# mcdiarmid/waveforms

Measured on AMD Instinct MI355X. Metric: SOQPSK-TG Msym/s mod+Viterbi-detect @8sps, higher is better.
Workload: dtype f64; 1 GPU; SOQPSK-TG 1e+07 symbols @8 sps, modulate + AWGN + PT matched filter + 4-state Viterbi detect (BASELINE configs[1]); waveform=soqpsk, sps=8, prbs=PN23, noise=Philox4x32-10 + Box-Muller (device), fuse=175, streams=1, detector_warmup_rows=16, detector_form=lanes (one chunk per lane), parallelism=independent trial blocks x1

## Files before the change

### include/wfhip.h

```cpp
#ifndef WFHIP_H
#define WFHIP_H

#include <stdint.h>

#ifdef __cplusplus
extern "C" {
#endif

typedef enum {
    WF_OK = 0,
    WF_ERR_VALUE = -1,
    WF_ERR_KEY = -2,
    WF_ERR_HIP = -3,
    WF_ERR_DEVICE = -4,
    WF_ERR_NOMEM = -5
} wf_status;

typedef struct wf_ctx wf_ctx;

const char *wf_version(void);
const char *wf_last_error_string(void);

int wf_ctx_create(int device, wf_ctx **out);
int wf_ctx_destroy(wf_ctx *ctx);
int wf_ctx_retire(wf_ctx *ctx);
int wf_ctx_check(wf_ctx *ctx, void *stream);
typedef enum {
    WF_OPT_CPM_FORM = 0,
    WF_OPT_CPM_CHUNK_CALLS = 1,
    WF_OPT_DET_REPAIR = 2,
    WF_OPT_DET_FINAL_VERIFY = 3,
    WF_OPT_ITERATION_SERVER = 4,
    WF_OPT_MCB_TAIL_PERMILLE = 5,
    WF_OPT_PIPE_RESERVE_CUS = 6,
    WF_OPT_CPM_SAMPLES_MIN_CALLS = 7,
    WF_OPT_SOFT_CHUNK_CALLS = 8,
    WF_OPT_CPM_SOFT_CHUNK_CALLS = 9,
    WF_OPT_COUNT = 10
} wf_option;
int wf_ctx_set_option(wf_ctx *ctx, int key, int64_t value);
int wf_ctx_get_option(wf_ctx *ctx, int key, int64_t *value);
int wf_ctx_forget_promises(wf_ctx *ctx);

int wf_lfsr_generate(wf_ctx *ctx, int degree, uint64_t mask, uint64_t state, uint64_t skip,
                     uint8_t *d_bits, int64_t n, uint64_t *h_state_out, void *stream);

int wf_fsm_encode(wf_ctx *ctx, const uint8_t *h_next, const int8_t *h_out, int columns, int states,
                  int card, const uint8_t *d_bits, int64_t nbits, int64_t i0, int state0,
                  int8_t *d_symbols, int *h_state_out, void *stream);

int wf_symbol_map(wf_ctx *ctx, int kind, const uint8_t *d_bits, int64_t n, int parity, int mem0,
                  int mem1, int8_t *d_symbols, void *stream);

int64_t wf_fir_out_len(int64_t nsym, int sps, int ntaps);
int wf_upsample_fir_f64(wf_ctx *ctx, const int8_t *d_symbols, int64_t nsym, const double *d_h,
                        int nh, const double *d_pulse, int ntaps, int sps, double *d_out,
                        void *stream);

int wf_phase_cexp_f64(wf_ctx *ctx, const double *d_freq, int64_t n, int sps, double phi0,
                      double revs_in, double *d_out_ri, double *d_revs_out, void *stream);
int wf_cpm_modulate_c128(wf_ctx *ctx, const int8_t *d_symbols, int64_t nsym, const double *d_h, int nh,
                         const double *d_pulse, int ntaps, int sps, double phi0, double *d_out_ri,
                         void *stream);
int wf_phase_modulate_f64(wf_ctx *ctx, const double *d_phase, int64_t n, double sens,
                          double *d_out_ri, void *stream);

int wf_awgn_c128(wf_ctx *ctx, const double *d_in_ri, int64_t n, double rot_re, double rot_im,
                 double sigma, uint64_t seed, uint64_t stream_id, uint64_t first_index,
                 double *d_out_ri, void *stream);

int wf_box_muller32_c128(wf_ctx *ctx, const uint32_t *d_words, int64_t n, double sigma, double *d_out_ri,
                         void *stream);

int wf_mf_bank_c128(wf_ctx *ctx, const double *d_r_ri, int64_t nsamp, const double *d_taps_ri,
                    int nfilt, int ntaps, int64_t first, int step, int64_t ncols,
                    double *d_out_ri, void *stream);

int wf_awgn_mf_bank_c128(wf_ctx *ctx, const double *d_signal_ri, int64_t nsamp, double rot_re, double rot_im,
                         double sigma, uint64_t seed, uint64_t stream_id, uint64_t first_index,
                         const double *d_taps_ri, int nfilt, int ntaps, int64_t first, int step,
                         int64_t ncols, double *d_out_ri, void *stream);

int wf_viterbi4_detect(wf_ctx *ctx, const double *d_mf_ri, int64_t ncalls, int differential,
                       int warmup, uint8_t *d_bits, int8_t *d_syms, double *d_state,
                       void *stream);
int wf_viterbi4_detect_window(wf_ctx *ctx, const double *d_mf_ri, int64_t ncalls, int length, int differential,
                              int warmup, uint8_t *d_bits, int8_t *d_syms, double *d_state, void *stream);
int64_t wf_viterbi4_window_state_bytes(void);
int wf_viterbi4_unmerged(wf_ctx *ctx, int64_t *h_count, int reset, void *stream);
int wf_viterbi_repaired(wf_ctx *ctx, int64_t *h_count, int reset, void *stream);
int wf_viterbi_cascaded(wf_ctx *ctx, int64_t *h_count, int reset, void *stream);

int wf_viterbi4_soft(wf_ctx *ctx, const double *d_rows, int64_t ncalls, int row_bytes, int differential, int warmup,
                     double *d_llr, uint8_t *d_bits, void *stream);
int wf_viterbi4_soft_geometry(wf_ctx *ctx, int64_t ncalls, int warmup, int64_t *h_geom);

int wf_viterbi4_soft_apriori(wf_ctx *ctx, const double *d_rows, int64_t ncalls, int row_bytes, int differential, int warmup,
                             const float *d_apriori, double apriori_scale, double *d_ext, uint8_t *d_bits, void *stream);

int wf_idd_windows(wf_ctx *ctx, const uint8_t *d_state, int64_t ncw, int64_t nrows, int32_t n_tx, int64_t P, int64_t row_offset,
                   const void *d_lock, int32_t L, int64_t G, int64_t *d_table, void *stream);
int wf_viterbi4_soft_apriori_windows(wf_ctx *ctx, const double *d_rows, int64_t ncalls, int row_bytes, int differential, int warmup,
                                     const float *d_apriori, double apriori_scale, const int64_t *d_windows, int64_t max_windows,
                                     double *d_ext, uint8_t *d_bits, void *stream);

int wf_viterbi4_detect_count(wf_ctx *ctx, const double *d_mf_ri, int64_t ncalls, int differential, int warmup,
                             uint8_t *d_bits, int8_t *d_syms, const uint8_t *d_ref_bits,
                             const int8_t *d_ref_syms, int skip, int64_t ncompare, int64_t *d_counts,
                             void *stream);
int64_t wf_viterbi4_state_bytes(int length);
int wf_viterbi4_iteration(wf_ctx *ctx, void *d_state, int length, int differential,
                          const double *d_mf3_ri, double *d_bits_out, double *d_syms_out,
                          void *stream);

int wf_viterbi4_iteration_host(wf_ctx *ctx, void *d_state, int length, int differential,
                               const double *h_mf3_ri, double *h_bits_out, double *h_syms_out, void *stream);
int wf_viterbi4_iteration_server_timing(wf_ctx *ctx, double *h_us4);
int wf_viterbi4_iteration_quiesce(wf_ctx *ctx);
int wf_viterbi4_state_read(wf_ctx *ctx, const void *d_state, int length, int64_t *h_calls, double *h_bi_history,
                           double *h_metrics, uint8_t *h_path, void *stream);

int wf_count_errors(wf_ctx *ctx, const int8_t *d_det_syms, const int8_t *d_ref_syms,
                    const uint8_t *d_det_bits, const uint8_t *d_ref_bits, int64_t m,
                    int64_t *d_counts, void *stream);

int wf_time_axis_f64(wf_ctx *ctx, int64_t n, double step, double *d_out, void *stream);

typedef struct {
    int64_t nsym;
    int sps;
    int degree;
    uint64_t mask, state, skip;
    int differential;
    const double *d_h;
    const double *d_pulse;
    int ntaps;
    const double *d_mf_taps;
    int mf_ntaps, mf_nfilt;
    int timing_offset;
    double sigma;
    uint64_t seed, stream_id;
    int warmup;
    int fuse;
    int event_slot;
    const double *d_mf_factor;
} wf_link_config;
#define WF_LINK_EVENT_SLOTS 64
#define WF_LINK_STAGES 8
int64_t wf_link_workspace_bytes(const wf_link_config *cfg);
int wf_link_run(wf_ctx *ctx, const wf_link_config *cfg, void *d_workspace, int64_t workspace_bytes,
                int64_t *d_counts, int64_t *h_compared, void *stream);
int wf_link_stage_ms(wf_ctx *ctx, int event_slot, float *h_ms);

int wf_link_join(wf_ctx *ctx, void *stream);

int wf_link_layout(const wf_link_config *cfg, int64_t *info8);

#define WF_LINK_STREAM_STATE_BYTES 512
int wf_mod_tile_geometry(int sps, int ntaps, int64_t nsym_total, int64_t *tile_len, int64_t *sym_per_tile,
                         int64_t *ntiles_total);
int64_t wf_link_stream_workspace_bytes(const wf_link_config *cfg, int64_t chunk_symbols);
int wf_link_stream_layout(const wf_link_config *cfg, int64_t chunk_symbols, int64_t chunk_index, int64_t *info8);
int wf_link_stream_chunk(wf_ctx *ctx, const wf_link_config *cfg, int64_t chunk_symbols, int64_t chunk_index,
                         void *d_state, void *d_workspace, int64_t workspace_bytes, int64_t *d_counts,
                         int64_t *h_compared, void *stream);
int wf_link_stream_chunk_phase(wf_ctx *ctx, const wf_link_config *cfg, int64_t chunk_symbols, int64_t chunk_index,
                               void *d_state, void *d_workspace, int64_t workspace_bytes, int64_t *d_counts,
                               int64_t *h_compared, int phases, void *stream);
int wf_link_stream_interior(const wf_link_config *cfg, int64_t chunk_symbols, int64_t chunk_index);
int wf_link_stream_steady(wf_ctx *ctx, const wf_link_config *cfg, int64_t chunk_symbols, void *d_state,
                          void *d_workspace, int64_t workspace_bytes, int64_t *d_counts, int64_t *h_compared,
                          void *stream);
int wf_link_stream_steady_phase(wf_ctx *ctx, const wf_link_config *cfg, int64_t chunk_symbols, void *d_state,
                                void *d_workspace, int64_t workspace_bytes, int64_t *d_counts, int64_t *h_compared,
                                int phases, void *stream);

typedef struct {
    int M;
    int p;
    int nh;
    int K[2];
    int Lp;
    int NC;
    int D;
} wf_cpm_detector_config;

int wf_cpm_mf_rows_c128(wf_ctx *ctx, const double *d_r_ri, int64_t nsamp, const double *d_templates_ri, int nh,
                        int nfilt, int ntm, int64_t start0, int sps, int64_t ncalls, double *d_rows_ri,
                        void *stream);

int wf_cpm_awgn_mf_rows_c128(wf_ctx *ctx, const double *d_signal_ri, int64_t nsamp, double rot_re, double rot_im,
                             double sigma, uint64_t seed, uint64_t stream_id, uint64_t first_index,
                             const double *d_templates_ri, int nh, int nfilt, int ntm, int64_t start0, int sps,
                             int64_t ncalls, double *d_rows_ri, void *stream);

#define WF_CPM_STATE_BYTES 16384
int wf_cpm_detector_form(wf_ctx *ctx, const wf_cpm_detector_config *det, int64_t ncalls, int warmup, int *info4);
int wf_cpm_viterbi_detect(wf_ctx *ctx, const wf_cpm_detector_config *det, const double *d_rot_cs,
                          const double *d_rows_ri, int64_t ncalls, int warmup, uint8_t *d_decisions,
                          void *d_state, void *stream);

int wf_cpm_viterbi_detect_samples(wf_ctx *ctx, const wf_cpm_detector_config *det, const double *d_rot_cs, const double *d_templates_ri,
                                  int nh, int nfilt, int ntm, const double *d_samples_ri, int64_t nsamp, int64_t start0, int sps,
                                  int64_t ncalls, int warmup, uint8_t *d_decisions, void *d_state, void *stream);

int wf_cpm_count_errors(wf_ctx *ctx, const uint8_t *d_decided_u, const int8_t *d_ref_alpha, int M, int64_t m,
                        int64_t *d_counts, void *stream);

int wf_cpm_soft(wf_ctx *ctx, const wf_cpm_detector_config *det, const double *d_rot_cs, const double *d_rows_ri,
                int64_t ncalls, int64_t first_call, int warmup, double *d_llr, uint8_t *d_bits, void *stream);
int wf_cpm_soft_geometry(wf_ctx *ctx, const wf_cpm_detector_config *det, int64_t ncalls, int warmup, int64_t *h_geom);

int wf_cpm_soft_apriori(wf_ctx *ctx, const wf_cpm_detector_config *det, const double *d_rot_cs, const double *d_rows_ri,
                        int64_t ncalls, int64_t first_call, int warmup, const float *d_apriori, double apriori_scale,
                        double *d_ext, uint8_t *d_bits, void *stream);

typedef struct wf_ldpc_code wf_ldpc_code;
int wf_ldpc_code_create(wf_ctx *ctx, int32_t n, int32_t m, const int32_t *h_check_ptr, const int32_t *h_edge_var,
                        int32_t nlayers, const int32_t *h_layer_ptr, int32_t n_tx, const int32_t *h_tx_var, int32_t k,
                        const int32_t *h_info_var, const uint64_t *h_parity_gen, wf_ldpc_code **out);
int wf_ldpc_code_free(wf_ldpc_code *code);
int wf_ldpc_encode(wf_ctx *ctx, const wf_ldpc_code *code, const uint8_t *d_info, int64_t ncw, uint8_t *d_tx, void *stream);
int wf_ldpc_decode(wf_ctx *ctx, const wf_ldpc_code *code, const double *d_llr, int64_t ncw, double scale, float alpha,
                   int max_iter, uint8_t *d_info_bits, float *d_post, int32_t *d_iters,
                   const uint8_t *d_ref_info, int64_t *d_counts, void *stream);
int wf_ldpc_decode_geometry(wf_ctx *ctx, const wf_ldpc_code *code, int64_t ncw, int64_t *h_geom);
int wf_ldpc_decode_ext(wf_ctx *ctx, const wf_ldpc_code *code, const double *d_llr, int64_t ncw, double scale, float alpha,
                       int max_iter, uint8_t *d_state, uint8_t *d_info_bits, float *d_post, int32_t *d_iters, float *d_ext,
                       int64_t ext_stride, float ext_clip, float ext_sat, void *stream);
int wf_ldpc_count(wf_ctx *ctx, const wf_ldpc_code *code, const uint8_t *d_info_bits, const uint8_t *d_ref_info,
                  const uint8_t *d_state, const int32_t *d_iters, int64_t ncw, int64_t *d_counts, void *stream);

int wf_frame_build(wf_ctx *ctx, const uint8_t *d_tx, int64_t ncw, int32_t n_tx, uint64_t marker, int32_t L, const uint8_t *d_pn,
                   uint8_t *d_out, void *stream);
int wf_frame_search(wf_ctx *ctx, const double *d_llr, int64_t nllr, uint64_t marker, int32_t L, int64_t P, void *d_lock,
                    double *d_folded, void *stream);
int wf_frame_gather(wf_ctx *ctx, const double *d_llr, int64_t nllr, const void *d_lock, int32_t L, int32_t n_tx, const uint8_t *d_pn,
                    int64_t ncw, double *d_out, void *stream);
int wf_frame_scatter(wf_ctx *ctx, const float *d_ext, int64_t ext_stride, const void *d_lock, uint64_t marker, int32_t L, int32_t n_tx,
// ... 50 lines not shown
```

### waveforms_amd/_hip.py

```python
from __future__ import annotations

import ctypes
import threading
from ctypes import POINTER, c_char_p, c_double, c_int, c_int64, c_uint64, c_void_p
from pathlib import Path

import numpy as np

import os

_LIB_PATH = Path(os.environ.get("WF_HIP_LIBRARY") or Path(__file__).resolve().parent / "csrc" / "libwfhip.so")

WF_ERR_VALUE, WF_ERR_KEY, WF_ERR_HIP, WF_ERR_DEVICE, WF_ERR_NOMEM = -1, -2, -3, -4, -5
WF_CPM_STATE_BYTES, WF_CPM_STREAM_STATE_BYTES = 16384, 20480
(WF_OPT_CPM_FORM, WF_OPT_CPM_CHUNK_CALLS, WF_OPT_DET_REPAIR, WF_OPT_DET_FINAL_VERIFY, WF_OPT_ITERATION_SERVER,
 WF_OPT_MCB_TAIL_PERMILLE, WF_OPT_PIPE_RESERVE_CUS, WF_OPT_CPM_SAMPLES_MIN_CALLS, WF_OPT_SOFT_CHUNK_CALLS,
 WF_OPT_CPM_SOFT_CHUNK_CALLS) = range(10)

_P = c_void_p
SIGNATURES = {
    "wf_version": (c_char_p, []),
    "wf_last_error_string": (c_char_p, []),
    "wf_ctx_create": (c_int, [c_int, POINTER(c_void_p)]),
    "wf_ctx_destroy": (c_int, [_P]),
    "wf_ctx_retire": (c_int, [_P]),
    "wf_ctx_check": (c_int, [_P, _P]),
    "wf_ctx_set_option": (c_int, [_P, c_int, c_int64]),
    "wf_ctx_get_option": (c_int, [_P, c_int, POINTER(c_int64)]),
    "wf_ctx_forget_promises": (c_int, [_P]),
    "wf_lfsr_generate": (c_int, [_P, c_int, c_uint64, c_uint64, c_uint64, _P, c_int64, POINTER(c_uint64), _P]),
    "wf_fsm_encode": (c_int, [_P, _P, _P, c_int, c_int, c_int, _P, c_int64, c_int64, c_int, _P, POINTER(c_int), _P]),
    "wf_symbol_map": (c_int, [_P, c_int, _P, c_int64, c_int, c_int, c_int, _P, _P]),
    "wf_fir_out_len": (c_int64, [c_int64, c_int, c_int]),
    "wf_upsample_fir_f64": (c_int, [_P, _P, c_int64, _P, c_int, _P, c_int, c_int, _P, _P]),
    "wf_phase_cexp_f64": (c_int, [_P, _P, c_int64, c_int, c_double, c_double, _P, _P, _P]),
    "wf_cpm_modulate_c128": (c_int, [_P, _P, c_int64, _P, c_int, _P, c_int, c_int, c_double, _P, _P]),
    "wf_phase_modulate_f64": (c_int, [_P, _P, c_int64, c_double, _P, _P]),
    "wf_time_axis_f64": (c_int, [_P, c_int64, c_double, _P, _P]),
    "wf_awgn_c128": (c_int, [_P, _P, c_int64, c_double, c_double, c_double, c_uint64, c_uint64, c_uint64, _P, _P]),
    "wf_box_muller32_c128": (c_int, [_P, _P, c_int64, c_double, _P, _P]),
    "wf_mf_bank_c128": (c_int, [_P, _P, c_int64, _P, c_int, c_int, c_int64, c_int, c_int64, _P, _P]),
    "wf_awgn_mf_bank_c128": (c_int, [_P, _P, c_int64, c_double, c_double, c_double, c_uint64, c_uint64, c_uint64, _P,
                                     c_int, c_int, c_int64, c_int, c_int64, _P, _P]),
    "wf_viterbi4_unmerged": (c_int, [_P, POINTER(c_int64), c_int, _P]),
    "wf_viterbi_repaired": (c_int, [_P, POINTER(c_int64), c_int, _P]),
    "wf_viterbi_cascaded": (c_int, [_P, POINTER(c_int64), c_int, _P]),
    "wf_viterbi4_detect_count": (c_int, [_P, _P, c_int64, c_int, c_int, _P, _P, _P, _P, c_int, c_int64, _P, _P]),
    "wf_viterbi4_detect": (c_int, [_P, _P, c_int64, c_int, c_int, _P, _P, _P, _P]),
    "wf_viterbi4_soft": (c_int, [_P, _P, c_int64, c_int, c_int, c_int, _P, _P, _P]),
    "wf_viterbi4_soft_geometry": (c_int, [_P, c_int64, c_int, POINTER(c_int64)]),
    "wf_viterbi4_soft_apriori": (c_int, [_P, _P, c_int64, c_int, c_int, c_int, _P, c_double, _P, _P, _P]),
    "wf_idd_windows": (c_int, [_P, _P, c_int64, c_int64, ctypes.c_int32, c_int64, c_int64, _P, ctypes.c_int32, c_int64, _P, _P]),
    "wf_viterbi4_soft_apriori_windows": (c_int, [_P, _P, c_int64, c_int, c_int, c_int, _P, c_double, _P, c_int64, _P, _P, _P]),
    "wf_viterbi4_detect_window": (c_int, [_P, _P, c_int64, c_int, c_int, c_int, _P, _P, _P, _P]),
    "wf_viterbi4_window_state_bytes": (c_int64, []),
    "wf_viterbi4_state_bytes": (c_int64, [c_int]),
    "wf_viterbi4_iteration": (c_int, [_P, _P, c_int, c_int, _P, _P, _P, _P]),
    "wf_viterbi4_iteration_host": (c_int, [_P, _P, c_int, c_int, _P, _P, _P, _P]),
    "wf_viterbi4_iteration_server_timing": (c_int, [_P, POINTER(ctypes.c_double)]),
    "wf_viterbi4_iteration_quiesce": (c_int, [_P]),
    "wf_link_join": (c_int, [_P, _P]),
    "wf_count_errors": (c_int, [_P, _P, _P, _P, _P, c_int64, _P, _P]),
    "wf_link_workspace_bytes": (c_int64, [_P]),
    "wf_link_run": (c_int, [_P, _P, _P, c_int64, _P, POINTER(c_int64), _P]),
    "wf_link_stage_ms": (c_int, [_P, c_int, POINTER(ctypes.c_float)]),
    "wf_link_layout": (c_int, [_P, POINTER(c_int64)]),
    "wf_mod_tile_geometry": (c_int, [c_int, c_int, c_int64, POINTER(c_int64), POINTER(c_int64), POINTER(c_int64)]),
    "wf_link_stream_workspace_bytes": (c_int64, [_P, c_int64]),
    "wf_link_stream_layout": (c_int, [_P, c_int64, c_int64, POINTER(c_int64)]),
    "wf_link_stream_chunk": (c_int, [_P, _P, c_int64, c_int64, _P, _P, c_int64, _P, POINTER(c_int64), _P]),
    "wf_link_stream_chunk_phase": (c_int, [_P, _P, c_int64, c_int64, _P, _P, c_int64, _P, POINTER(c_int64), c_int, _P]),
    "wf_link_stream_interior": (c_int, [_P, c_int64, c_int64]),
    "wf_link_stream_steady": (c_int, [_P, _P, c_int64, _P, _P, c_int64, _P, POINTER(c_int64), _P]),
    "wf_link_stream_steady_phase": (c_int, [_P, _P, c_int64, _P, _P, c_int64, _P, POINTER(c_int64), c_int, _P]),
    "wf_welch_scratch_doubles": (c_int64, [c_int64, c_int]),
    "wf_welch_psd_c128": (c_int, [_P, _P, c_int64, c_int, c_double, _P, c_double, _P, _P, _P]),
    "wf_phase_tree_f64": (c_int, [_P, _P, c_int64, c_int, c_int, c_int, c_double, _P, _P]),
    "wf_eye_traces_c128": (c_int, [_P, _P, _P, c_int64, c_int, c_int, c_double, _P, _P, _P, _P]),
    "wf_cpm_mf_rows_c128": (c_int, [_P, _P, c_int64, _P, c_int, c_int, c_int, c_int64, c_int, c_int64, _P, _P]),
    "wf_cpm_awgn_mf_rows_c128": (c_int, [_P, _P, c_int64, c_double, c_double, c_double, c_uint64, c_uint64, c_uint64, _P, c_int, c_int,
                                         c_int, c_int64, c_int, c_int64, _P, _P]),
    "wf_viterbi4_state_read": (c_int, [_P, _P, c_int, POINTER(c_int64), _P, _P, _P, _P]),
    "wf_cpm_detector_form": (c_int, [_P, _P, c_int64, c_int, POINTER(c_int)]),
    "wf_cpm_viterbi_detect": (c_int, [_P, _P, _P, _P, c_int64, c_int, _P, _P, _P]),
    "wf_cpm_viterbi_detect_samples": (c_int, [_P, _P, _P, _P, c_int, c_int, c_int, _P, c_int64, c_int64, c_int, c_int64, c_int, _P, _P, _P]),
    "wf_cpm_count_errors": (c_int, [_P, _P, _P, c_int, c_int64, _P, _P]),
    "wf_cpm_soft": (c_int, [_P, _P, _P, _P, c_int64, c_int64, c_int, _P, _P, _P]),
    "wf_cpm_soft_geometry": (c_int, [_P, _P, c_int64, c_int, POINTER(c_int64)]),
    "wf_cpm_soft_apriori": (c_int, [_P, _P, _P, _P, c_int64, c_int64, c_int, _P, c_double, _P, _P, _P]),
    "wf_ldpc_code_create": (c_int, [_P, ctypes.c_int32, ctypes.c_int32, _P, _P, ctypes.c_int32, _P, ctypes.c_int32, _P, ctypes.c_int32,
                                    _P, _P, POINTER(c_void_p)]),
    "wf_ldpc_code_free": (c_int, [_P]),
    "wf_ldpc_encode": (c_int, [_P, _P, _P, c_int64, _P, _P]),
    "wf_ldpc_decode": (c_int, [_P, _P, _P, c_int64, c_double, ctypes.c_float, c_int, _P, _P, _P, _P, _P, _P]),
    "wf_ldpc_decode_geometry": (c_int, [_P, _P, c_int64, POINTER(c_int64)]),
    "wf_ldpc_decode_ext": (c_int, [_P, _P, _P, c_int64, c_double, ctypes.c_float, c_int, _P, _P, _P, _P, _P, c_int64, ctypes.c_float,
                           ctypes.c_float, _P]),
    "wf_ldpc_count": (c_int, [_P, _P, _P, _P, _P, _P, c_int64, _P, _P]),
    "wf_frame_build": (c_int, [_P, _P, c_int64, ctypes.c_int32, c_uint64, ctypes.c_int32, _P, _P, _P]),
    "wf_frame_search": (c_int, [_P, _P, c_int64, c_uint64, ctypes.c_int32, c_int64, _P, _P, _P]),
    "wf_frame_gather": (c_int, [_P, _P, c_int64, _P, ctypes.c_int32, ctypes.c_int32, _P, c_int64, _P, _P]),
    "wf_frame_scatter": (c_int, [_P, _P, c_int64, _P, c_uint64, ctypes.c_int32, ctypes.c_int32, _P, c_int64, ctypes.c_float, _P, c_int64, _P]),
    "wf_cpm_link_workspace_bytes": (c_int64, [_P]),
    "wf_cpm_link_run": (c_int, [_P, _P, _P, c_int64, _P, POINTER(c_int64), _P]),
    "wf_cpm_link_layout": (c_int, [_P, POINTER(c_int64)]),
    "wf_cpm_link_form": (c_int, [_P, _P, POINTER(c_int)]),
    "wf_cpm_link_stream_workspace_bytes": (c_int64, [_P, c_int64]),
    "wf_cpm_link_stream_layout": (c_int, [_P, c_int64, c_int64, POINTER(c_int64)]),
    "wf_cpm_link_stream_chunk": (c_int, [_P, _P, c_int64, c_int64, _P, _P, c_int64, _P, POINTER(c_int64), _P]),
    "wf_cpm_link_stream_chunk_phase": (c_int, [_P, _P, c_int64, c_int64, _P, _P, c_int64, _P, POINTER(c_int64), c_int, _P]),
}


class CPMDetectorConfig(ctypes.Structure):

    _fields_ = [("M", c_int), ("p", c_int), ("nh", c_int), ("K", c_int * 2), ("Lp", c_int), ("NC", c_int), ("D", c_int)]


class CPMLinkConfig(ctypes.Structure):

    _fields_ = [
        ("nsym", c_int64), ("sps", c_int), ("degree", c_int), ("mask", c_uint64), ("state", c_uint64), ("skip", c_uint64),
        ("mapper_kind", c_int), ("det", CPMDetectorConfig), ("d_h", c_void_p), ("d_pulse", c_void_p), ("ntaps", c_int),
        ("d_templates", c_void_p), ("d_rot_cs", c_void_p), ("sigma", c_double), ("seed", c_uint64), ("stream_id", c_uint64),
        ("warmup", c_int), ("skip_head", c_int), ("event_slot", c_int), ("fuse", c_int),
    ]


class LinkConfig(ctypes.Structure):

    _fields_ = [
        ("nsym", c_int64), ("sps", c_int), ("degree", c_int), ("mask", c_uint64), ("state", c_uint64),
        ("skip", c_uint64), ("differential", c_int), ("d_h", c_void_p), ("d_pulse", c_void_p),
        ("ntaps", c_int), ("d_mf_taps", c_void_p), ("mf_ntaps", c_int), ("mf_nfilt", c_int),
        ("timing_offset", c_int), ("sigma", c_double), ("seed", c_uint64), ("stream_id", c_uint64),
        ("warmup", c_int), ("fuse", c_int), ("event_slot", c_int), ("d_mf_factor", c_void_p),
    ]


_lib = None
_lock = threading.RLock()
_ctxs: dict[int, int] = {}


def lib() -> ctypes.CDLL:
    global _lib
    if _lib is None:
        with _lock:
            if _lib is None:
# ... 154 lines not shown
```

### waveforms_amd/csrc/wf_common.h

```cpp
#pragma once
#include <hip/hip_runtime.h>
#include <stdint.h>

#include <atomic>
#include <map>
#include <mutex>
#include <vector>
#include <string>

#include "../../include/wfhip.h"

#define WF_WAVE 64

void wf_set_error(const char *fmt, ...);

#define WF_HIP(call)                                                                     \
    do {                                                                                 \
        hipError_t e_ = (call);                                                          \
        if (e_ != hipSuccess) {                                                          \
            wf_set_error("%s failed: %s (%s:%d)", #call, hipGetErrorString(e_), __FILE__, \
                         __LINE__);                                                      \
            return WF_ERR_HIP;                                                           \
        }                                                                                \
    } while (0)
// ... 3 lines not shown
        if (!(cond)) {                 \
            wf_set_error(__VA_ARGS__); \
            return WF_ERR_VALUE;       \
        }                              \
    } while (0)

#define WF_LAUNCH_CHECK() WF_HIP(hipGetLastError())

enum { WF_FAULT_SCAN_TIMEOUT = 1u, WF_FAULT_LIVE_TABLE = 2u };

struct wf_lfsr_tables {
    uint64_t host[64][64];
    uint64_t *dev = nullptr;
    uint64_t f_even = 0, f_odd = 0, f_m2 = 0, f_m1 = 0;
    bool f_ready = false;
};

struct wf_ctx {
    int device = 0;
    int cus = 256;
    int64_t opt[WF_OPT_COUNT] = {0};
    uint64_t *d_scan = nullptr;
    size_t scan_words = 0;
    unsigned *d_fault = nullptr;
    unsigned *h_fault = nullptr;
    uint8_t *d_tables = nullptr;
    uint8_t h_tables_cache[2048] = {0};
    int tables_cached = 0;
    hipEvent_t tables_event = nullptr;
    hipStream_t tables_stream = nullptr;
    bool tables_pending = false;
    uint64_t *d_fsm_scratch = nullptr;
    size_t fsm_scratch_words = 0;
    int *h_small = nullptr;
    int *d_small = nullptr;
    std::map<uint64_t, wf_lfsr_tables *> lfsr;
    double *d_mod_scratch = nullptr;
    size_t mod_scratch_words = 0;
    double *d_vit_edge = nullptr;
    size_t vit_edge_words = 0;
    unsigned long long *d_vit_unmerged = nullptr;
    hipEvent_t *events = nullptr;
    void *pipe_stream = nullptr;
    void *pipe_stream2 = nullptr;
    void *pipe_pro = nullptr, *pipe_main = nullptr;
    hipEvent_t pipe_call = nullptr, pipe_pro_done = nullptr;
    hipEvent_t pipe_front = nullptr, pipe_done[2] = {nullptr, nullptr};
    bool pipe_done_valid[2] = {false, false};
    int pipe_set = 0;
    std::map<uint64_t, uint32_t> promises;
    std::mutex promises_lock;
    double *h_iter = nullptr;
    double *d_iter = nullptr;
    void *h_mailbox = nullptr;
    void *d_mailbox = nullptr;
    void *iter_stream = nullptr;
    const void *iter_last_state = nullptr;
    std::atomic_flag iter_lock = ATOMIC_FLAG_INIT;
    bool iter_closing = false;
};

static inline hipStream_t wf_stream(void *s) { return reinterpret_cast<hipStream_t>(s); }

int wf_ctx_reserve_scan(wf_ctx *ctx, size_t words);
int wf_ctx_reserve_fsm(wf_ctx *ctx, size_t words);
int wf_ctx_reserve_mod(wf_ctx *ctx, size_t words);
int wf_iter_server_stop(wf_ctx *ctx);
int wf_ctx_reserve_vit(wf_ctx *ctx, size_t words);

struct lfsr_emit_args;
int wf_lfsr_generate_dyn(wf_ctx *ctx, int degree, uint64_t mask, uint64_t state, uint64_t skip,
                         const uint64_t *d_dyn_skip, uint8_t *d_bits, int64_t n, uint64_t *h_state_out, void *stream,
                         const struct lfsr_emit_args *emit = nullptr);
int wf_lfsr_generate_map(wf_ctx *ctx, int degree, uint64_t mask, uint64_t state, uint64_t skip, uint8_t *d_bits, int64_t nbits,
                         int map_kind, int8_t *d_symbols, void *stream);
int wf_soqpsk_prbs_encode(wf_ctx *ctx, int degree, uint64_t mask, uint64_t state, uint64_t skip, const uint8_t *h_next,
                          const int8_t *h_out, uint8_t *d_bits, int64_t n, int8_t *d_symbols, void *stream, void *mid_event = nullptr);
int wf_awgn_mf_bank_dyn(wf_ctx *ctx, const double *d_signal_ri, int64_t nsamp, double rot_re, double rot_im,
                        double sigma, uint64_t seed, uint64_t stream_id, uint64_t first_index,
                        const uint64_t *d_dyn_index, const double *d_taps_ri, int nfilt, int ntaps, int64_t first,
                        int step, int64_t ncols, double *d_out_ri, void *stream, int pack_par0 = -1);
int wf_viterbi4_detect_packed(wf_ctx *ctx, const double *d_rows4, int64_t ncalls, int differential, int warmup,
                              uint8_t *d_bits, int8_t *d_syms, double *d_state, void *stream);
int wf_cpm_modulate_window(wf_ctx *ctx, const int8_t *d_symbols, int64_t sym_origin, int64_t nloc, int64_t nsym_total,
                           const double *d_h, int nh, const double *d_pulse, int ntaps, int sps, double phi0,
                           int64_t tile_lo, int64_t ntiles, double *d_out_ri, int64_t out_origin,
                           const uint64_t *d_q_in, uint64_t *d_q_out, int64_t q_out_tile, void *stream);
struct wf_mcb_opts {
    const double *pam_factor = nullptr;
    bool cpm_paired = false;
    int runs_hint = 0;
    int scratch_slot = -1;
};
int wf_mod_chan_bank_packed(wf_ctx *ctx, const int8_t *d_symbols, int64_t nsym, const double *d_h, int nh,
                            const double *d_pulse, int ntaps, int sps, double phi0, const double *d_mf_taps, double rot_re,
                            double rot_im, double sigma, uint64_t seed, uint64_t stream_id, uint64_t first_index,
                            int64_t first, int64_t ncols, int pack_par0, double *d_rows4, void *stream, int mf_ntaps = 0,
                            const wf_mcb_opts *opts = nullptr, int stage = 3);
int wf_mod_chan_bank_window(wf_ctx *ctx, const int8_t *d_symbols, int64_t sym_origin, int64_t nloc, int64_t nsym_total,
                            const double *d_h, int nh, const double *d_pulse, int ntaps, int sps, double phi0,
                            int64_t tile_lo, int64_t ntiles, const uint64_t *d_q_in, uint64_t *d_q_out, int64_t q_out_tile,
                            const double *d_mf_taps, double rot_re, double rot_im, double sigma, uint64_t seed,
                            uint64_t stream_id, uint64_t first_index, const uint64_t *d_dyn_index, int64_t first,
                            int64_t k_lo, int64_t ncols, int pack_par0, double *d_rows4, void *stream, int cpm_nf = 0, int cpm_nh = 1,
                            int stage = 3, int mf_ntaps = 0, const wf_mcb_opts *opts = nullptr);
int wf_mod_chan_bank_applies(int64_t nsym, int nh, int ntaps, int sps, int mf_ntaps, int64_t first);
int wf_link_join_internal(wf_ctx *ctx, void *stream);
int wf_mod_chan_cpm_rows_applies(int64_t nsym, int nh, int ntaps, int sps, int nfilt, int ntm, int64_t start0);
int wf_mod_chan_cpm_rows(wf_ctx *ctx, const int8_t *d_symbols, int64_t nsym, const double *d_h, int nh, const double *d_pulse,
                         int ntaps, int sps, double phi0, const double *d_templates, int nfilt, int ntm, int64_t start0,
                         double rot_re, double rot_im, double sigma, uint64_t seed, uint64_t stream_id, int64_t ncalls,
                         double *d_rows, void *stream, const wf_mcb_opts *opts = nullptr);
int wf_mod_chan_samples_applies(int64_t nsym, int nh, int ntaps, int sps);
int wf_mod_chan_samples(wf_ctx *ctx, const int8_t *d_symbols, int64_t nsym, const double *d_h, int nh, const double *d_pulse, int ntaps,
                        int sps, double phi0, double rot_re, double rot_im, double sigma, uint64_t seed, uint64_t stream_id,
                        uint64_t first_index, double *d_out_ri, void *stream);
int wf_mod_chan_samples_window(wf_ctx *ctx, const int8_t *d_symbols, int64_t sym_origin, int64_t nloc, int64_t nsym_total, const double *d_h, int nh,
                               const double *d_pulse, int ntaps, int sps, double phi0, int64_t tile_lo, int64_t ntiles, const uint64_t *d_q_in,
                               uint64_t *d_q_out, int64_t q_out_tile, double rot_re, double rot_im, double sigma, uint64_t seed, uint64_t stream_id,
                               uint64_t first_index, double *d_out_ri, int64_t out_origin, int64_t out_hi, void *stream);
int wf_promise_verified(wf_ctx *ctx, int kind, const void *const *d_ptrs, const size_t *nbytes, int nptrs, void *stream,
                        bool (*check)(const unsigned char *const *host, const size_t *nbytes, const void *arg), const void *arg, const char *what);
int wf_fsm_encode_core(wf_ctx *ctx, const uint8_t *h_next, const int8_t *h_out, int columns, int states, int card,
                       const uint8_t *d_bits, int64_t nbits, int64_t i0, int state0, const int *d_state_in,
                       int8_t *d_symbols, int *h_state_out, int *d_state_at, int64_t at_index, void *stream);

static inline int wf_grid_for(int64_t work_items, int per_block, int max_blocks)
{
    int64_t b = (work_items + per_block - 1) / per_block;
    if (b < 1) b = 1;
    if (b > max_blocks) b = max_blocks;
    return (int)b;
}

#ifdef __HIPCC__
__device__ __forceinline__ int wf_lane() { return threadIdx.x & (WF_WAVE - 1); }

__device__ __forceinline__ void wf_lds_barrier()
{
    asm volatile("s_waitcnt lgkmcnt(0)\n\ts_barrier" ::: "memory");
}

typedef double wf_v2d __attribute__((ext_vector_type(2)));
__device__ __forceinline__ void wf_store16_nt(double2 *p, double2 v)
{
    wf_v2d t = {v.x, v.y};
    __builtin_nontemporal_store(t, reinterpret_cast<wf_v2d *>(p));
}
__device__ __forceinline__ double2 wf_load16_nt(const double2 *p)
{
    const wf_v2d t = __builtin_nontemporal_load(reinterpret_cast<const wf_v2d *>(p));
    return make_double2(t.x, t.y);
}

template <int CTRL, int ROW_MASK>
__device__ __forceinline__ double wf_dpp_f64(double v)
{
    constexpr bool BC = ROW_MASK == 0xf;
    const long long b = __double_as_longlong(v);
    const int lo = __builtin_amdgcn_update_dpp(0, (int)b, CTRL, ROW_MASK, 0xf, BC);
    const int hi = __builtin_amdgcn_update_dpp(0, (int)(b >> 32), CTRL, ROW_MASK, 0xf, BC);
    return __longlong_as_double(((long long)hi << 32) | (unsigned)lo);
}

__device__ __forceinline__ double wf_wave_incl_scan(double v)
{
    v += wf_dpp_f64<0x111, 0xf>(v);
    v += wf_dpp_f64<0x112, 0xf>(v);
    v += wf_dpp_f64<0x114, 0xf>(v);
    v += wf_dpp_f64<0x118, 0xf>(v);
    v += wf_dpp_f64<0x142, 0xa>(v);
    v += wf_dpp_f64<0x143, 0xc>(v);
    return v;
}

// ... 328 lines not shown
```

### waveforms_amd/csrc/wf_ctx.hip

```cpp
#include <stdarg.h>
#include <stdio.h>

#include "wf_common.h"

static thread_local char g_err[512] = "";

void wf_set_error(const char *fmt, ...)
{
    va_list ap;
    va_start(ap, fmt);
    vsnprintf(g_err, sizeof(g_err), fmt, ap);
    va_end(ap);
}

extern "C" const char *wf_version(void) { return "waveforms-amd 0.1.0 (gfx950)"; }
extern "C" const char *wf_last_error_string(void) { return g_err; }

extern "C" int wf_ctx_create(int device, wf_ctx **out)
{
    WF_REQUIRE(out != nullptr, "wf_ctx_create: out is NULL");
    int ndev = 0;
    WF_HIP(hipGetDeviceCount(&ndev));
    WF_REQUIRE(device >= 0 && device < ndev, "wf_ctx_create: device %d of %d", device, ndev);
    WF_HIP(hipSetDevice(device));
// ... 16 lines not shown
}

extern "C" int wf_ctx_destroy(wf_ctx *c)
{
    if (!c) return WF_OK;
    (void)hipSetDevice(c->device);
    (void)wf_iter_server_stop(c);
    (void)hipDeviceSynchronize();
    for (auto &kv : c->lfsr) {
        if (kv.second->dev) (void)hipFree(kv.second->dev);
        delete kv.second;
    }
    if (c->events) {
        for (int k = 0; k < WF_LINK_EVENT_SLOTS * (WF_LINK_STAGES + 1); ++k) (void)hipEventDestroy(c->events[k]);
        delete[] c->events;
    }
    if (c->pipe_front) (void)hipEventDestroy(c->pipe_front);
    for (int k = 0; k < 2; ++k)
        if (c->pipe_done[k]) (void)hipEventDestroy(c->pipe_done[k]);
    if (c->pipe_stream) (void)hipStreamDestroy(static_cast<hipStream_t>(c->pipe_stream));
    if (c->pipe_stream2) (void)hipStreamDestroy(static_cast<hipStream_t>(c->pipe_stream2));
    if (c->pipe_pro) (void)hipStreamDestroy(static_cast<hipStream_t>(c->pipe_pro));
    if (c->pipe_main) (void)hipStreamDestroy(static_cast<hipStream_t>(c->pipe_main));
    if (c->pipe_call) (void)hipEventDestroy(c->pipe_call);
    if (c->pipe_pro_done) (void)hipEventDestroy(c->pipe_pro_done);
    if (c->d_scan) (void)hipFree(c->d_scan);
    if (c->d_fsm_scratch) (void)hipFree(c->d_fsm_scratch);
    if (c->d_mod_scratch) (void)hipFree(c->d_mod_scratch);
    if (c->d_vit_edge) (void)hipFree(c->d_vit_edge);
    if (c->d_vit_unmerged) (void)hipFree(c->d_vit_unmerged);
    if (c->d_fault) (void)hipFree(c->d_fault);
    if (c->h_fault) (void)hipHostFree(c->h_fault);
    if (c->d_tables) (void)hipFree(c->d_tables);
    if (c->tables_event) (void)hipEventDestroy(c->tables_event);
    if (c->d_small) (void)hipFree(c->d_small);
    if (c->h_small) (void)hipHostFree(c->h_small);
    if (c->h_iter) (void)hipHostFree(c->h_iter);
    if (c->iter_stream) (void)hipStreamDestroy(static_cast<hipStream_t>(c->iter_stream));
    if (c->h_mailbox) (void)hipHostFree(c->h_mailbox);
    delete c;
    return WF_OK;
}

extern "C" int wf_ctx_retire(wf_ctx *c)
{
    if (!c) return WF_OK;
    (void)hipSetDevice(c->device);
    (void)wf_iter_server_stop(c);
    if (c->pipe_stream) (void)hipStreamSynchronize(static_cast<hipStream_t>(c->pipe_stream));
    if (c->pipe_stream2) (void)hipStreamSynchronize(static_cast<hipStream_t>(c->pipe_stream2));
    if (c->pipe_pro) (void)hipStreamSynchronize(static_cast<hipStream_t>(c->pipe_pro));
    if (c->pipe_main) (void)hipStreamSynchronize(static_cast<hipStream_t>(c->pipe_main));
    return WF_OK;
}

int wf_link_join_internal(wf_ctx *c, void *stream)
{
    if (!c) return WF_OK;
    for (int k = 0; k < 2; ++k)
        if (c->pipe_done_valid[k]) WF_HIP(hipStreamWaitEvent(wf_stream(stream), c->pipe_done[k], 0));
    return WF_OK;
}

extern "C" int wf_link_join(wf_ctx *c, void *stream)
{
    WF_REQUIRE(c != nullptr, "wf_link_join: ctx is NULL");
    return wf_link_join_internal(c, stream);
}

extern "C" int wf_ctx_set_option(wf_ctx *c, int key, int64_t value)
{
    WF_REQUIRE(c != nullptr, "wf_ctx_set_option: ctx is NULL");
    WF_REQUIRE(key >= 0 && key < WF_OPT_COUNT, "wf_ctx_set_option: unknown option %d", key);
    bool ok = true;
    switch (key) {
    case WF_OPT_CPM_FORM: ok = value >= 0 && value <= 2; break;
    case WF_OPT_CPM_CHUNK_CALLS: ok = value >= 0 && value <= 8192; break;
    case WF_OPT_DET_REPAIR: case WF_OPT_DET_FINAL_VERIFY: case WF_OPT_ITERATION_SERVER: ok = value == 0 || value == 1; break;
    case WF_OPT_MCB_TAIL_PERMILLE: ok = value >= -1 && value <= 16000; break;
    case WF_OPT_PIPE_RESERVE_CUS: ok = value >= -1 && value <= 128; break;
    case WF_OPT_CPM_SAMPLES_MIN_CALLS: ok = value == 0 || (value >= 4096 && value <= ((int64_t)1 << 40)); break;
    case WF_OPT_SOFT_CHUNK_CALLS: ok = value >= 0 && value <= 8192; break;
    case WF_OPT_CPM_SOFT_CHUNK_CALLS: ok = value >= 0 && value <= 8192; break;
    }
    WF_REQUIRE(ok, "wf_ctx_set_option: value %lld outside the range of option %d", (long long)value, key);
    c->opt[key] = value;
    return WF_OK;
}

extern "C" int wf_ctx_get_option(wf_ctx *c, int key, int64_t *value)
{
    WF_REQUIRE(c != nullptr && value != nullptr, "wf_ctx_get_option: NULL argument");
    WF_REQUIRE(key >= 0 && key < WF_OPT_COUNT, "wf_ctx_get_option: unknown option %d", key);
    *value = c->opt[key];
    return WF_OK;
}

extern "C" int wf_ctx_check(wf_ctx *c, void *stream)
{
    WF_REQUIRE(c != nullptr, "wf_ctx_check: ctx is NULL");
    {
        const int rj = wf_link_join_internal(c, stream);
        if (rj) return rj;
    }
    WF_HIP(hipMemcpyAsync(c->h_fault, c->d_fault, sizeof(unsigned), hipMemcpyDeviceToHost,
                          wf_stream(stream)));
    WF_HIP(hipStreamSynchronize(wf_stream(stream)));
    unsigned f = *c->h_fault;
    if (f) {
        WF_HIP(hipMemsetAsync(c->d_fault, 0, sizeof(unsigned), wf_stream(stream)));
        wf_set_error("device fault word 0x%x (bit0 = scan hand-off timeout, bit1 = malformed live-window table)", f);
        return WF_ERR_DEVICE;
    }
    return WF_OK;
}

int wf_promise_verified(wf_ctx *c, int kind, const void *const *d_ptrs, const size_t *nbytes, int nptrs, void *stream,
                        bool (*check)(const unsigned char *const *host, const size_t *nbytes, const void *arg), const void *arg, const char *what)
{
    uint64_t key = 1469598103934665603ull;
    auto mix = [&](uint64_t v) {
        for (int b = 0; b < 8; ++b) {
            key ^= (v >> (8 * b)) & 0xFFull;
            key *= 1099511628211ull;
        }
    };
    mix((uint64_t)kind);
    for (int i = 0; i < nptrs; ++i) {
        WF_REQUIRE(d_ptrs[i] != nullptr && nbytes[i] > 0 && nbytes[i] <= (1u << 16), "%s: operand %d is NULL or larger than 64 KB", what, i);
        mix((uint64_t)reinterpret_cast<uintptr_t>(d_ptrs[i]));
        mix((uint64_t)nbytes[i]);
    }
    std::lock_guard<std::mutex> guard(c->promises_lock);
    auto it = c->promises.find(key);
    if (it != c->promises.end()) {
        ++it->second;
        return WF_OK;
    }
    hipStreamCaptureStatus cap = hipStreamCaptureStatusNone;
    (void)hipStreamIsCapturing(wf_stream(stream), &cap);
    if (cap != hipStreamCaptureStatusNone) {
        WF_REQUIRE(it != c->promises.end(), "%s: cannot be verified inside a stream capture — run the configuration once eagerly first", what);
        return WF_OK;
    }
    std::vector<std::vector<unsigned char>> host(nptrs);
    std::vector<const unsigned char *> hp(nptrs);
    for (int i = 0; i < nptrs; ++i) {
        host[i].resize(nbytes[i]);
        WF_HIP(hipMemcpyAsync(host[i].data(), d_ptrs[i], nbytes[i], hipMemcpyDeviceToHost, wf_stream(stream)));
        hp[i] = host[i].data();
    }
    WF_HIP(hipStreamSynchronize(wf_stream(stream)));
    if (!check(hp.data(), nbytes, arg)) {
        if (it != c->promises.end()) c->promises.erase(it);
        wf_set_error("%s", what);
        return WF_ERR_VALUE;
    }
    c->promises[key] = 1;
    return WF_OK;
}

extern "C" int wf_ctx_forget_promises(wf_ctx *c)
{
    WF_REQUIRE(c != nullptr, "wf_ctx_forget_promises: ctx is NULL");
    std::lock_guard<std::mutex> guard(c->promises_lock);
    c->promises.clear();
// ... 55 lines not shown
```

### waveforms_amd/csrc/wf_modulate.hip

```cpp
#include <type_traits>

#include "wf_common.h"

#ifndef MOD_THREADS
#define MOD_THREADS 256
#endif
#ifndef MOD_ROWS
#define MOD_ROWS 16
#endif
#define MOD_WAVES (MOD_THREADS / WF_WAVE)
#define MOD_MASK ((1ull << 62) - 1)
#define MOD_MAX_PART 40
#define MOD_SCAN_TAPS 2048
#define MOD_SCAN_PER 16
#define MOD_MAX_NH 8

struct mod_params {
    int64_t nsym, out_len, ntiles;
    int sps, ntaps, nh, c, rs;
    int spt;
    int dsh;
    int npart;
    int nhead;
    double sps_d, inv_sps, phi0_turns;
// ... 380 lines not shown
    const int q0 = (2 * t + P.c) / sps;
    const int r0 = (2 * t + P.c) - q0 * sps;
    const int wrap = (r0 + 1 == sps) ? 1 : 0;
    const int r1 = wrap ? 0 : r0 + 1;
    const bool any_wrap = (sps & 1) != 0 || (P.c & 1) != 0;
    const double *Gcum = scratch + MOD_OFF_GCUM(P.ntiles);
    double Q0[JMAX], Q1[JMAX];
#pragma unroll
    for (int j = 0; j < JMAX; ++j) {
        const int k0 = r0 + j * sps, k1 = r1 + j * sps;
        Q0[j] = Gcum[k0 < P.ntaps ? k0 : P.ntaps - 1];
        Q1[j] = Gcum[k1 < P.ntaps ? k1 : P.ntaps - 1];
    }
    const double sec_per_unit = 128.0 * P.inv_sps, sec_phi0 = 128.0 * P.phi0_turns;
    const int l_top0p1 = (q0 - cq) + JMAX;
    const int win = MOD_ROWS * sym_per_row + JMAX + 2;
    int *s_pi = reinterpret_cast<int *>(s_amp + ((win + 1) & ~1));
    const double T = scratch[0];
    const double Th_a = T * hvec[0], Th_b = P.nh > 1 ? T * hvec[1] : 0.0;
    const int lpart = JMAX - cq - P.dsh;

    for (int64_t tile = blockIdx.x; tile < P.ntiles; tile += gridDim.x) {
        auto kt = KA0;
        asm volatile("" : "+s"(kt));
        const auto &P = kt->P;
        const int8_t *__restrict__ const symbols = kt->symbols;
        const double *__restrict__ const hvec = kt->hvec;
        double *__restrict__ const out = kt->out;
        const uint64_t *Wq = reinterpret_cast<const uint64_t *>(kt->scratch + MOD_OFF_P + P.ntiles);
        int tp = t;
        asm volatile("" : "+v"(tp));
        const int64_t tile_g = P.tile_lo + tile;
        const int64_t tile_base = tile_g * tile_len;
        const int64_t sym_base = tile_base / sps;
        const int64_t mp1_lo = sym_base + cq - JMAX + 1;
        const bool full_tile = tile_base >= P.out_origin && tile_base + tile_len <= P.out_hi;
        wf_lds_barrier();
        mod_stage_window<MANY_H>(symbols, hvec, P, mp1_lo - 1, win, s_amp, s_pi, s_wtot, tp);
        const double W = (double)Wq[tile] * 0x1.0p-62 * P.sps_d;
        const int ref_a = s_pi[lpart], ref_b = P.nh > 1 ? s_pi[win + 1 + lpart] : 0;
#pragma unroll 2
        for (int u = 0; u < MOD_ROWS; ++u) {
            double2 e0 = make_double2(0.0, 0.0), e1 = e0;
            if (active) {
                double ra, rb;
                mod_pair_phase<JMAX>(Q0, Q1, &s_amp[l_top0p1 + u * sym_per_row], &s_pi[(q0 - cq) + u * sym_per_row], wrap, any_wrap,
                                     MANY_H ? P.nh : (P.nh > 1 ? 2 : 1), win + 1, ref_a, ref_b, W, Th_a, Th_b, P.sps_d, P.inv_sps, ra, rb,
                                     MANY_H ? &s_pi[lpart] : nullptr, hvec, T);
                wf_sincos_sectors(s_cis, fma(ra, sec_per_unit, sec_phi0), &e0.y, &e0.x);
                wf_sincos_sectors(s_cis, fma(rb, sec_per_unit, sec_phi0), &e1.y, &e1.x);
            }
            double2 *xw = s_xp + wave * (2 * WF_WAVE);
            xw[2 * lane] = e0;
            xw[2 * lane + 1] = e1;
            __builtin_amdgcn_fence(__ATOMIC_RELEASE, "wavefront");
            __builtin_amdgcn_wave_barrier();
            __builtin_amdgcn_fence(__ATOMIC_ACQUIRE, "wavefront");
            const double2 xa = xw[lane], xb = xw[WF_WAVE + lane];
            const int col = wave * (2 * WF_WAVE) + lane;
            const int64_t na = tile_base + (int64_t)u * P.rs + col, nb = na + WF_WAVE;
            double2 *o = reinterpret_cast<double2 *>(out);
            if (full_tile) {
                if (FULLROW || col < P.rs) wf_store16_nt(o + (na - P.out_origin), xa);
                if (FULLROW || col + WF_WAVE < P.rs) wf_store16_nt(o + (nb - P.out_origin), xb);
            } else {
                if ((FULLROW || col < P.rs) && na >= P.out_origin && na < P.out_hi) wf_store16_nt(o + (na - P.out_origin), xa);
                if ((FULLROW || col + WF_WAVE < P.rs) && nb >= P.out_origin && nb < P.out_hi) wf_store16_nt(o + (nb - P.out_origin), xb);
            }
        }
    }
}

struct mcb_params {
    double rot_re, rot_im, sigma;
    uint64_t seed, stream_id, pair0;
    const uint64_t *dyn_index;
    int64_t k_lo, k_hi;
    int kshift;
    int d;
    int pack_par0;
    int cpm_nh;
    int mf_ntaps;
    int n_long, run_long;
};

template <int SPS>
struct mcb_geom {
    static constexpr int L2 = (SPS % 2 == 0) ? SPS : 2 * SPS;
    static constexpr int RS = (2 * MOD_THREADS / L2) * L2;
    static constexpr int CPR = RS / SPS;
    static constexpr int NT = SPS + 1;
    static constexpr int RING = 2 * RS;
    static constexpr int GROUPS = RING / SPS;
    static constexpr int GS = SPS + 1;
    static constexpr int SLOTS = GROUPS * GS + 16;
};
#define MCB_RING 1024
#define MCB_SLOTS (MCB_RING + MCB_RING / 8 + 16)
static_assert(mcb_geom<8>::RING == MCB_RING && mcb_geom<8>::SLOTS == MCB_SLOTS, "SPS = 8 geometry");

template <int CTRL>
__device__ __forceinline__ double mcb_quad_bcast(double v)
{
    const long long b = __double_as_longlong(v);
    const int lo = __builtin_amdgcn_update_dpp(0, (int)b, CTRL, 0xf, 0xf, true);
    const int hi = __builtin_amdgcn_update_dpp(0, (int)(b >> 32), CTRL, 0xf, 0xf, true);
    return __longlong_as_double(((long long)hi << 32) | (unsigned)lo);
}

#ifndef WF_MCB_WAVES
#define WF_MCB_WAVES 4
#endif
#ifndef WF_MCB_CPM_WAVES
#define WF_MCB_CPM_WAVES 4
#endif
#ifndef WF_MCB_UNROLL
#define WF_MCB_UNROLL 2
#endif
#ifndef WF_MCB_SECTION_OFF
#define WF_MCB_SECTION_OFF 0
#endif
#define WF_MCB_PRIO 3
struct mcb_kargs {
    const int8_t *symbols;
    const double *hvec, *pulse, *scratch, *mf_taps;
    double *rows;
    mod_params P;
    mcb_params Q;
};
typedef const __attribute__((address_space(4))) mcb_kargs *mcb_kptr;

template <int SPS, int SH = 4>
struct mcb_pam_geom {
    static constexpr int NT = 9 * SPS + 1;
    static constexpr int PG = SH * SPS;
    static constexpr int OPLEN = (SH - 1) * SPS + NT;
    static constexpr int NK = SH == 4 ? (2 * OPLEN + 3) / 4 : (OPLEN + 3) / 4;
    static constexpr int NKW = NK / 4;
    static constexpr int QSH = (mcb_geom<SPS>::CPR & 1) ? 3 : 0;
    static constexpr int OPROWS = (mcb_geom<SPS>::CPR + QSH + SH - 1) / SH;
    static constexpr int XLEN = NT + 1;
    static constexpr int LASTREAD = SH == 4 ? OPLEN + 1 : 4 * NK;
    static constexpr int MIRROR = (PG * (OPROWS - 1) + LASTREAD - QSH * SPS - mcb_geom<SPS>::RS + 7) & ~7;
    static constexpr int EXT = mcb_geom<SPS>::RING + MIRROR;
    static constexpr int SLOTS = EXT + EXT / PG + 1;
    static_assert(NK % 4 == 1, "wave 0 takes exactly one k-step more than the others");
    static_assert((mcb_geom<SPS>::RS - QSH * SPS) % PG == 0 && PG % (SH == 4 ? 8 : 16) == 0, "operand rows start on the pad grid in both rows of the ring");
    static_assert((SH == 4 ? (((mcb_geom<SPS>::CPR - QSH) & 1) == 0 && OPROWS <= 16) : OPROWS <= 8), "one B operand set for both row parities");
};
static_assert(mcb_pam_geom<8>::NT == 73 && mcb_pam_geom<8>::NK == 49 && mcb_pam_geom<8>::XLEN == 74 && mcb_pam_geom<8>::OPROWS == 16 && mcb_pam_geom<8>::MIRROR == 72, "SPS = 8 PAM geometry");
static_assert(mcb_pam_geom<10>::NT == 91 && mcb_pam_geom<10>::NK == 61 && mcb_pam_geom<10>::OPROWS == 14 && mcb_pam_geom<10>::MIRROR == 104, "SPS = 10 PAM geometry");
static_assert(mcb_pam_geom<8, 8>::NK == 33 && mcb_pam_geom<8, 8>::OPROWS == 8 && mcb_pam_geom<8, 8>::MIRROR == 72 && mcb_pam_geom<10, 8>::NK == 41 && mcb_pam_geom<10, 8>::OPROWS == 7 && mcb_pam_geom<10, 8>::MIRROR == 104, "factored PAM geometry");
#define MCB_PAM_NT(sps) (9 * (sps) + 1)
static inline int mcb_pam_slots(int sps, bool factored)
{
    return factored ? (sps == 8 ? mcb_pam_geom<8, 8>::SLOTS : mcb_pam_geom<10, 8>::SLOTS) : (sps == 8 ? mcb_pam_geom<8>::SLOTS : mcb_pam_geom<10>::SLOTS);
}
template <int JMAX, int CPMNF, int SPS = 8>
__global__ __launch_bounds__(MOD_THREADS, CPMNF == 0 ? WF_MCB_WAVES : (CPMNF < 0 ? 3 : (JMAX <= 4 ? WF_MCB_CPM_WAVES : 2))) void mod_chan_bank_kernel(const int8_t *__restrict__ symbols_,
                                                                     const double *__restrict__ hvec_,
                                                                     const double *__restrict__ pulse_,
                                                                     const double *__restrict__ scratch_,
                                                                     const double *__restrict__ mf_taps_,
                                                                     double *__restrict__ rows_, mod_params P_, mcb_params Q_)
{
    mcb_kptr const KA0 = (mcb_kptr)__builtin_amdgcn_kernarg_segment_ptr();
// ... 140 lines not shown
        const int s_sh = mf_i >> 1, kf = mf_i & 1;
        const int nt = Q.mf_ntaps;
        const double *bf = mf_taps + kf * nt;
#pragma unroll
        for (int n = 0; n <= GP::NKW; ++n) {
            const int kk = 4 * n + wave_u;
            const int cc = 4 * kk + mf_kq - SPS * s_sh;
            double v = 0.0;
            if (cc >= 0 && cc < nt && (n < GP::NKW || wave_u == 0)) v = bf[nt - 1 - cc];
            bpam[n] = v;
        }
        for (int k = t; k < RSLOTS; k += MOD_THREADS) s_ring[k] = make_double2(0.0, 0.0);
    } else if constexpr (PAM) {
        const int s_sh = mf_i >> 2, o_sl = mf_i & 3;
        const int nt = Q.mf_ntaps;
        const bool odd_col = ((Q.pack_par0 + s_sh - Q.kshift) & 1) != 0;
        const int f = o_sl < 2 ? 1 : (o_sl == 2 ? 0 : 2);
        const bool want_im = o_sl == 1 || (o_sl == 2 && odd_col) || (o_sl == 3 && !odd_col);
        const double2 *tg = reinterpret_cast<const double2 *>(mf_taps) + f * nt;
#pragma unroll
        for (int n = 0; n <= GP::NKW; ++n) {
            const int kk = 4 * n + wave_u;
            const int cc = 4 * kk + mf_kq - 2 * SPS * s_sh;
            double v = 0.0;
            if (cc >= 0 && cc < 2 * nt && (n < GP::NKW || wave_u == 0)) {
                const double2 tp = tg[nt - 1 - (cc >> 1)];
                v = want_im ? ((cc & 1) ? tp.y : tp.x) : ((cc & 1) ? tp.x : -tp.y);
            }
            bpam[n] = v;
        }
        for (int k = t; k < RSLOTS; k += MOD_THREADS) s_ring[k] = make_double2(0.0, 0.0);
    }

    typedef __attribute__((address_space(3))) wf_v2d *mcb_lds2;
    constexpr bool RINGPK = CPMNF == 0 && (SPS == 8 || JMAX <= 4);
    unsigned ring_pk_a = 0, ring_pk_b = 0;
    static_assert(!RINGPK || (((MOD_ROWS * CPR + JMAX + 2 + 1) & ~1) * 8 + RSLOTS * 16 + 2 * (MOD_ROWS * CPR + JMAX + 3) * 4 + 12 * 1024) < 65536,
                  "packed ring addresses need the workgroup's LDS below 64 KB");
    if constexpr (RINGPK) {
        const unsigned base = (unsigned)(uintptr_t)(__attribute__((address_space(3))) char *)s_ring;
        for (int par = 0; par < 2; ++par) {
            int ia = (par ? RS : 0) + 2 * t - Q.d;
            ia += ia < 0 ? G::RING : 0;
            const int ib = ia + 1 == G::RING ? 0 : ia + 1;
            ring_pk_a |= (base + 16u * (unsigned)(ia + ia / PG)) << (16 * par);
            ring_pk_b |= (base + 16u * (unsigned)(ib + ib / PG)) << (16 * par);
        }
    }
    const int bx = (int)blockIdx.x;
    const int lt0 = bx < Q.n_long ? bx * Q.run_long : Q.n_long * Q.run_long + (bx - Q.n_long);
    const int lt1_ = bx < Q.n_long ? lt0 + Q.run_long : lt0 + 1;
    const int lt1 = lt1_ < (int)P.ntiles ? lt1_ : (int)P.ntiles;
    if (lt0 == 0 && P.tile_lo == 0)
        for (int k = t; k < RSLOTS; k += MOD_THREADS) s_ring[k] = make_double2(0.0, 0.0);
    bool run_first = true;
    for (int ltile = lt0; ltile < lt1; ++ltile, run_first = false) {
        const bool run_last = ltile + 1 == lt1;
        auto kt = KA0;
        MCB_FRESH(kt);
        const auto &P = kt->P;
        const auto &Q = kt->Q;
        const int8_t *__restrict__ const symbols = kt->symbols;
        const double *__restrict__ const hvec = kt->hvec;
        double *__restrict__ const rows = kt->rows;
        const int64_t tile = P.tile_lo + ltile;
        const int64_t tile_base = tile * tile_len;
        const int64_t sym_base = tile_base / sps;
        const int cq_t = P.c / sps;
        const int64_t mp1_lo = sym_base + cq_t - JMAX + 1;
        const int lpart = JMAX - cq_t - P.dsh;
        const bool full_tile = tile_base + tile_len <= P.out_len;
        const int64_t klo64 = Q.k_lo - sym_base, khi64 = Q.k_hi - sym_base;
        const int klo = klo64 < -(1 << 20) ? -(1 << 20) : (int)klo64, khi = khi64 > (1 << 20) ? (1 << 20) : (int)khi64;
        char *const tile_rows4 = reinterpret_cast<char *>(rows) + 32 * (sym_base - Q.k_lo);
        wf_lds_barrier();
        unsigned lane0 = 0u;
        asm volatile("" : "+v"(lane0));
        int tp = (int)__builtin_amdgcn_mbcnt_hi(~0u, __builtin_amdgcn_mbcnt_lo(~0u, lane0)) + 64 * wave_u;
        mod_stage_window(symbols, hvec, P, mp1_lo - 1, win, s_amp, s_pi, s_wtot, tp);
        const uint64_t pair_t = Q.pair0 + (Q.dyn_index ? (*Q.dyn_index >> 1) : 0ull) + (uint64_t)(tile_base >> 1) + (uint64_t)tp;
        const uint64_t *Wq = reinterpret_cast<const uint64_t *>(kt->scratch + MOD_OFF_P + P.ntiles);
        const double W = (double)Wq[ltile] * 0x1.0p-62 * P.sps_d;
        const int ref_a = s_pi[lpart], ref_b = P.nh > 1 ? s_pi[win + 1 + lpart] : 0;
        auto bank_row = [&](int rho) __attribute__((always_inline)) {
            const int kr = CPR * rho + mq - Q.kshift;
            const int64_t k = sym_base + kr;
            const bool k_ok = kr >= klo && kr < khi && (CPR == 64 || mq < CPR);
            const int grp = ((rho & 1) ? CPR : 0) + (CPR == 64 ? mq : (mq < CPR ? mq : 0));
            const bool odd = ((Q.pack_par0 + kr + (int)(sym_base & 1)) & 1) != 0;
            if constexpr (PAIRED && USE_MFMA) {
                const int mqi = 32 * (wave_u >> 1) + 2 * mf_i + (wave_u & 1);
                const int grp_i = ((rho & 1) ? 64 : 0) + mqi;
                const double2 *xs = s_ring + 9 * grp_i + mf_kq;
                mcb_d4 accx = {0.0, 0.0, 0.0, 0.0}, accy = accx;
#pragma unroll
                for (int kk = 0; kk < 3; ++kk) {
                    double2 a = kk < 2 ? xs[4 * kk] : xs[9 - mf_kq];
                    if (kk == 2 && mf_kq >= 1) a = make_double2(0.0, 0.0);
                    accx = __builtin_amdgcn_mfma_f64_16x16x4f64(a.x, bmat[kk], accx, 0, 0, 0);
                    accy = __builtin_amdgcn_mfma_f64_16x16x4f64(a.y, bmat[3 + kk], accy, 0, 0, 0);
                }
                const int pj = mf_i & 7, imj = mf_i >> 3;
#pragma unroll
                for (int reg = 0; reg < 4; ++reg) {
                    const int isym = mf_kq + 4 * reg;
                    const int kr_i = 64 * rho + 32 * (wave_u >> 1) + 2 * isym + (wave_u & 1) - Q.kshift;
                    const double u = accx[reg], v = accy[reg];
                    const double first = u + v, dd = u - v;
                    const double second = imj ? -dd : dd;
                    if (kr_i >= klo && kr_i < khi) {
                        double *o = rows + ((sym_base + kr_i) - Q.k_lo) * (2 * NF) + imj;
                        __builtin_nontemporal_store(first, &o[2 * pj]);
                        __builtin_nontemporal_store(second, &o[2 * (15 - pj)]);
                    }
                }
            } else if constexpr (USE_MFMA) {
                const int mqi = 32 * (wave_u >> 1) + 2 * mf_i + (wave_u & 1);
                const int grp_i = ((rho & 1) ? 64 : 0) + mqi;
                const double *xa = ring_d + 2 * (9 * grp_i) + ((mf_kq & 1) ? 0 : 1) + 2 * (mf_kq >> 1);
                mcb_d4 acc0 = {0.0, 0.0, 0.0, 0.0}, acc1 = acc0;
#pragma unroll
                for (int kk = 0; kk < 5; ++kk) {
                    double a = kk < 4 ? xa[4 * kk] : xa[2 * 9 - 2 * (mf_kq >> 1)];
                    if (kk == 4 && mf_kq >= 2) a = 0.0;
                    acc0 = __builtin_amdgcn_mfma_f64_16x16x4f64(a, bmat[kk], acc0, 0, 0, 0);
                    acc1 = __builtin_amdgcn_mfma_f64_16x16x4f64(a, bmat[5 + kk], acc1, 0, 0, 0);
                }
                const int jo = mf_i;
#pragma unroll
                for (int reg = 0; reg < 4; ++reg) {
                    const int isym = mf_kq + 4 * reg;
                    const int kr_i = 64 * rho + 32 * (wave_u >> 1) + 2 * isym + (wave_u & 1) - Q.kshift;
                    if (kr_i >= klo && kr_i < khi) {
                        double *o = rows + ((sym_base + kr_i) - Q.k_lo) * (2 * NF) + jo;
                        __builtin_nontemporal_store(acc0[reg], &o[0]);
                        __builtin_nontemporal_store(acc1[reg], &o[16]);
                    }
                }
            } else if constexpr (PAM2) {
                const int ri = mf_i & 7;
                const int S0 = ((rho & 1) ? RS - GP::QSH * SPS : 0) + PG * (GP::OPROWS < 8 && ri >= GP::OPROWS ? 0 : ri);
                const double *xa = ring_d + 2 * (S0 + S0 / PG + 4 * wave_u + mf_kq) + (mf_i >> 3);
                mcb_d4 acc = {0.0, 0.0, 0.0, 0.0};
#pragma unroll
                for (int n = 0; n < GP::NKW; ++n)
                    acc = __builtin_amdgcn_mfma_f64_16x16x4f64(xa[2 * (16 * n + 16 * n / PG)], bpam[n], acc, 0, 0, 0);
                if (wave_u == 0) acc = __builtin_amdgcn_mfma_f64_16x16x4f64(xa[2 * (16 * GP::NKW + 16 * GP::NKW / PG)], bpam[GP::NKW], acc, 0, 0, 0);
#pragma unroll
                for (int reg = 0; reg < 4; ++reg) s_part[(4 * wave_u + reg) * 64 + (t & 63)] = acc[reg];
            } else if constexpr (PAM) {
                const int S0 = ((rho & 1) ? RS - GP::QSH * SPS : 0) + PG * (GP::OPROWS < 16 && mf_i >= GP::OPROWS ? 0 : mf_i);
                const double *xa = ring_d + 2 * (S0 + S0 / PG + 2 * wave_u + (mf_kq >> 1)) + ((mf_kq & 1) ? 0 : 1);
                mcb_d4 acc = {0.0, 0.0, 0.0, 0.0};
#pragma unroll
                for (int n = 0; n < GP::NKW; ++n)
                    acc = __builtin_amdgcn_mfma_f64_16x16x4f64(xa[2 * (8 * n + 8 * n / PG)], bpam[n], acc, 0, 0, 0);
                if (wave_u == 0) acc = __builtin_amdgcn_mfma_f64_16x16x4f64(xa[2 * (8 * GP::NKW + 8 * GP::NKW / PG)], bpam[GP::NKW], acc, 0, 0, 0);
#pragma unroll
                for (int reg = 0; reg < 4; ++reg) s_part[(4 * wave_u + reg) * 64 + (t & 63)] = acc[reg];
            } else if constexpr (PAIRED) {
                const int q = mp >> 1, pl = mp & 1;
                const double *xb = ring_d + 2 * (9 * grp) + pl;
                const int col = Q.cpm_nh == 2 ? (int)((sym_base + kr) & 1) : 0;
                const double2 *tb_ = s_taps + (col * NF + q) * 9;
                double sc = 0.0, ss = 0.0;
#pragma unroll
                for (int j = 0; j < 9; ++j) {
                    const double xv = xb[2 * (j < 8 ? j : 9)];
                    const double2 tp = tb_[j];
                    sc = fma(xv, tp.x, sc);
                    ss = fma(xv, tp.y, ss);
                }
                const double got = mcb_quad_bcast<0xB1>(ss);
                const double first = pl ? sc - got : sc + got;
                const double second = pl ? sc + got : sc - got;
                if (k_ok) {
                    double *o = rows + 2 * (k - Q.k_lo) * NF + pl;
                    __builtin_nontemporal_store(first, &o[2 * q]);
                    __builtin_nontemporal_store(second, &o[2 * (NF - 1 - q)]);
                }
            } else if constexpr (CPMNF != 0) {
                constexpr int FPT = CPMNF / 4;
                const double2 *xb = s_ring + 9 * grp;
                const int col = Q.cpm_nh == 2 ? (int)((sym_base + kr) & 1) : 0;
                const double2 *tb_ = s_taps + (col * CPMNF + FPT * mp) * 9;
                double zr[FPT], zi[FPT];
#pragma unroll
                for (int f = 0; f < FPT; ++f) zr[f] = zi[f] = 0.0;
#pragma unroll
                for (int j = 0; j < 9; ++j) {
                    const double2 xv = xb[j < 8 ? j : 9];
#pragma unroll
                    for (int f = 0; f < FPT; ++f) {
                        const double2 tp = tb_[f * 9 + j];
                        zr[f] = fma(xv.x, tp.x, fma(xv.y, tp.y, zr[f]));
                        zi[f] = fma(-xv.x, tp.y, fma(xv.y, tp.x, zi[f]));
                    }
                }
                if (k_ok) {
                    double *o = rows + 2 * ((k - Q.k_lo) * CPMNF + FPT * mp);
#pragma unroll
                    for (int f = 0; f < FPT; ++f) {
                        __builtin_nontemporal_store(zr[f], &o[2 * f]);
                        __builtin_nontemporal_store(zi[f], &o[2 * f + 1]);
                    }
                }
            } else if (sym_taps_i != 0) {
                const double *xb = ring_d + 2 * (G::GS * grp) + (mp & 1);
                const double *tapc = s_tapc + NT * (4 * ((CPR & 1) ? (int)odd : odd_l) + mp);
                const double x_first = xb[0];
                double S = x_first * tapc[0], U = x_first;
#pragma unroll NT <= 11 ? NT - 1 : 5
                for (int j = 1; j < NT; ++j) {
                    const double x = xb[2 * (j < SPS ? j : G::GS)];
                    S = fma(x, tapc[j], S);
                    U += x;
                }
                const double T = S + mcb_quad_bcast<0xB1>(S);
                const double val = (mp == 0 || mp == 3) ? U : T;
                if (k_ok) {
                    *reinterpret_cast<double *>(tile_rows4 + (int64_t)(32 * (CPR * rho - Q.kshift)) + (unsigned)(32 * mq + 8 * slot_l)) = val;
                }
            } else {
                const int f = mp < 2 ? 1 : (mp == 2 ? 0 : 2);
                const bool imag = mp == 1 || (mp == 2 && odd) || (mp == 3 && !odd);
                const double2 *xb = s_ring + G::GS * grp;
                double acc = 0.0;
#pragma unroll 1
                for (int j = 0; j < NT; ++j) {
                    const double2 x = xb[j < SPS ? j : G::GS];
                    const double2 tp = s_taps[f * NT + (NT - 1 - j)];
                    acc = imag ? fma(x.x, tp.y, fma(x.y, tp.x, acc)) : fma(x.x, tp.x, fma(-x.y, tp.y, acc));
                }
                if (k_ok) *reinterpret_cast<double *>(tile_rows4 + (int64_t)(32 * (CPR * rho - Q.kshift)) + (unsigned)(32 * mq + 8 * mp)) = acc;
            }
        };
        auto bank_reduce = [&](int rho) __attribute__((always_inline)) {
            if constexpr (PAM2) {
                const int ln = t & 63, tc = 16 * wave_u + (ln >> 2), p4 = ln & 3;
                const int ri = tc >> 3, reg = (ri >> 2) + 2 * (p4 & 1), lsrc = 2 * (tc & 7) + (p4 >> 1) + 16 * (ri & 3);
                const double *pp = s_part + reg * 64 + lsrc;
                const double v = ((pp[0] + pp[4 * 64]) + pp[8 * 64]) + pp[12 * 64];
                const double y0r = mcb_quad_bcast<0x00>(v), y0i = mcb_quad_bcast<0x55>(v), y1r = mcb_quad_bcast<0xAA>(v), y1i = mcb_quad_bcast<0xFF>(v);
                const int col = tc - ((rho & 1) ? GP::QSH : 0);
                const int kr = CPR * rho + col - Q.kshift;
                const int odd_c = (Q.pack_par0 + kr + (int)(sym_base & 1)) & 1;
                const double *gt = s_gt + 16 * odd_c + 4 * p4;
                const double out = fma(gt[3], y1i, fma(gt[2], y1r, fma(gt[1], y0i, gt[0] * y0r)));
                if (kr >= klo && kr < khi && (CPR == 64 || (col >= 0 && col < CPR)))
                    *reinterpret_cast<double *>(tile_rows4 + (int64_t)(32 * (CPR * rho - Q.kshift)) + (unsigned)(32 * col + 8 * p4)) = out;
            } else if constexpr (PAM) {
                const int ln = t & 63;
                const double *pp = s_part + (4 * 0 + wave_u) * 64 + ln;
                const double v = ((pp[0] + pp[4 * 64]) + pp[8 * 64]) + pp[12 * 64];
                const int col = 16 * wave_u + (ln >> 2) - ((rho & 1) ? GP::QSH : 0);
                const int kr = CPR * rho + col - Q.kshift;
                if (kr >= klo && kr < khi && (CPR == 64 || (col >= 0 && col < CPR))) rows[4 * ((sym_base + kr) - Q.k_lo) + (ln & 3)] = v;
            }
        };
        auto row_step = [&](const int u, auto parc) __attribute__((always_inline)) {
            const bool EXTRA = u >= MOD_ROWS;
            double2 x0 = make_double2(0.0, 0.0), x1 = x0;
            bool have_next = true;
            if ((!EXTRA || wave_u == 0) && active) {
            auto next_tile_refs = [&](double &Wn, int &na, int &nb) __attribute__((always_inline)) {
                have_next = ltile + 1 < P.ntiles;
                Wn = have_next ? (double)Wq[ltile + 1] * 0x1.0p-62 * P.sps_d : 0.0;
                na = s_pi[lpart + MOD_ROWS * sym_per_row];
                nb = P.nh > 1 ? s_pi[win + 1 + lpart + MOD_ROWS * sym_per_row] : 0;
            };
            double ra, rb;
            double2 e0, e1;
            constexpr bool LOADS_FIRST = (CPMNF <= 0 && (SPS != 10 || JMAX == 9)) || (CPMNF == 32 && JMAX <= 4);
            double am_[JMAX];
            int pi0_ = 0, pi1_ = 0;
            if constexpr (!LOADS_FIRST) {
                double Wu = W;
                int refu_a = ref_a, refu_b = ref_b;
                if (EXTRA) next_tile_refs(Wu, refu_a, refu_b);
                mod_pair_phase<JMAX>(Q0, Q1, &s_amp[l_top0p1 + u * sym_per_row], &s_pi[(q0 - cq) + u * sym_per_row], wrap, any_wrap, P.nh,
                                     win + 1, refu_a, refu_b, Wu, Th_a, Th_b, (double)SPS, 1.0 / (double)SPS, ra, rb);
                wf_sincos_sectors_pos(s_cis, fma(ra, sec_per_unit, sec_phi0), &e0.y, &e0.x);
                wf_sincos_sectors_pos(s_cis, fma(rb, sec_per_unit, sec_phi0), &e1.y, &e1.x);
            } else if constexpr (!(WF_MCB_SECTION_OFF & 4)) {
                const double *ap = &s_amp[l_top0p1 + u * sym_per_row];
                const int *pp = &s_pi[(q0 - cq) + u * sym_per_row];
#pragma unroll
                for (int j = 0; j < JMAX; ++j) am_[j] = ap[-1 - j];
                pi0_ = pp[0];
                if (P.nh > 1) pi1_ = pp[win + 1];
            }
            double g[4];
            {
                uint32_t k0 = (uint32_t)Q.seed, k1 = (uint32_t)(Q.seed >> 32);
                asm volatile("" : "+s"(k0), "+s"(k1));
                __builtin_amdgcn_s_setprio(0);
                wf_gaussian_two_il<true, decltype(tb), CPMNF == 0 && SPS == 8, WF_MCB_SECTION_OFF & 3>(pair_t + (uint64_t)(u * (RS / 2)), Q.stream_id, ((uint64_t)k1 << 32) | k0, Q.sigma, tb, g);
                __builtin_amdgcn_s_setprio(WF_MCB_PRIO);
            }
            if constexpr (LOADS_FIRST && (WF_MCB_SECTION_OFF & 4)) {
                e0 = make_double2(1.0, 0.0);
                e1 = make_double2(0.0, 1.0);
            } else if constexpr (LOADS_FIRST) {
                double acc0 = 0.0, acc1 = 0.0;
#pragma unroll
                for (int j = 0; j < JMAX; ++j) {
                    acc0 = fma(Q0[j], am_[j], acc0);
                    acc1 = fma(Q1[j], am_[j], acc1);
                }
                double b0;
                if (!EXTRA) {
                    b0 = fma((double)(pi0_ - ref_a), Th_a, W);
                    if (P.nh > 1) b0 = fma((double)(pi1_ - ref_b), Th_b, b0);
                } else {
                    double Wn;
                    int na, nb;
                    next_tile_refs(Wn, na, nb);
// ... 262 lines not shown
    } while (0)
    if (J <= 4) MOD_LAUNCH(4);
    else if (J <= 9) MOD_LAUNCH(9);
    else if (J <= 17) MOD_LAUNCH(17);
    else MOD_LAUNCH(33);
#undef MOD_LAUNCH
    WF_LAUNCH_CHECK();
    return WF_OK;
}

extern "C" int wf_cpm_modulate_c128(wf_ctx *ctx, const int8_t *d_symbols, int64_t nsym, const double *d_h,
                                    int nh, const double *d_pulse, int ntaps, int sps, double phi0,
                                    double *d_out_ri, void *stream)
{
    WF_REQUIRE(ctx && d_h && d_pulse && d_out_ri, "wf_cpm_modulate_c128: NULL argument");
    WF_REQUIRE(nsym >= 0 && (nsym == 0 || d_symbols), "wf_cpm_modulate_c128: bad symbols");
    WF_REQUIRE(sps >= 2 || nsym == 0, "could not broadcast input array from shape (%lld,) into shape (%lld,)",
               (long long)nsym, (long long)(nsym - 1));
    WF_REQUIRE(sps >= 1 && sps <= 256 && nh >= 1 && ntaps >= 1, "wf_cpm_modulate_c128: sps %d nh %d ntaps %d", sps, nh, ntaps);
    WF_REQUIRE((reinterpret_cast<uintptr_t>(d_out_ri) & 15) == 0, "wf_cpm_modulate_c128: d_out alignment");
    WF_HIP(hipSetDevice(ctx->device));
    mod_params P;
    if (!mod_setup(P, nsym, nh, ntaps, sps, phi0, MOD_MAX_NH)) return 1;
    return mod_launch(ctx, P, d_symbols, d_h, d_pulse, d_out_ri, nullptr, nullptr, stream);
}

int wf_mod_chan_bank_window(wf_ctx *ctx, const int8_t *d_symbols, int64_t sym_origin, int64_t nloc, int64_t nsym_total,
                            const double *d_h, int nh, const double *d_pulse, int ntaps, int sps, double phi0,
                            int64_t tile_lo, int64_t ntiles, const uint64_t *d_q_in, uint64_t *d_q_out, int64_t q_out_tile,
                            const double *d_mf_taps, double rot_re, double rot_im, double sigma, uint64_t seed,
                            uint64_t stream_id, uint64_t first_index, const uint64_t *d_dyn_index, int64_t first,
                            int64_t k_lo, int64_t ncols, int pack_par0, double *d_rows4, void *stream, int cpm_nf, int cpm_nh,
                            int stage, int mf_ntaps, const wf_mcb_opts *opts)
{
    const wf_mcb_opts none{};
    const wf_mcb_opts &O = opts ? *opts : none;
    WF_REQUIRE(ctx && d_symbols && d_h && d_pulse && d_mf_taps && d_rows4, "wf_mod_chan_bank: NULL argument");
    if (cpm_nf != 0 && cpm_nf != 4 && cpm_nf != 16) return 1;
    if (cpm_nf && cpm_nh != 1 && cpm_nh != 2) return 1;
    if (!(phi0 * (128.0 / (2.0 * M_PI)) >= 1.0)) return 1;
    if (mf_ntaps <= 0) mf_ntaps = sps + 1;
    const bool pam = cpm_nf == 0 && mf_ntaps != sps + 1;
    if (pam && ((sps != 8 && sps != 10) || mf_ntaps < 3 || mf_ntaps > MCB_PAM_NT(sps) || (mf_ntaps & 1) == 0)) return 1;
    WF_REQUIRE((reinterpret_cast<uintptr_t>(d_rows4) & 15) == 0 && (reinterpret_cast<uintptr_t>(d_mf_taps) & 15) == 0,
               "wf_mod_chan_bank: device pointers must be 16-byte aligned");
    mod_params P;
    const bool sps_ok = sps == 8 || (cpm_nf == 0 && (sps == 10 || sps == 20));
    if (!sps_ok || (first_index & 1) || first < 0 || first >= sps || ncols < 1 || k_lo < 0) return 1;
    const int rs_want = sps == 8 ? mcb_geom<8>::RS : (sps == 10 ? mcb_geom<10>::RS : mcb_geom<20>::RS);
    if (!mod_setup(P, nsym_total, nh, ntaps, sps, phi0) || P.rs != rs_want) return 1;
    const int J = (ntaps + sps - 1) / sps;
    if (J > 9) return 1;
    if (cpm_nf == 0 && (sps != 10 || J > 4) && ((sps & 1) || (P.c & 1))) return 1;
    WF_REQUIRE(first + (k_lo + ncols - 1) * (int64_t)sps < P.out_len, "wf_mod_chan_bank: columns run past the burst");
    if (ntiles < 0) ntiles = P.ntiles;
    WF_REQUIRE(tile_lo >= 0 && ntiles >= 1 && tile_lo + ntiles <= P.ntiles && ntiles < (int64_t)1 << 31, "wf_mod_chan_bank: bad tile window");
    P.sym_origin = sym_origin;
    P.nloc = nloc;
    P.tile_lo = tile_lo;
    P.ntiles = ntiles;
    P.q_out_tile = q_out_tile;
    WF_HIP(hipSetDevice(ctx->device));
    if (stage & 1) {
        int rc = mod_launch_carries(ctx, P, d_symbols, d_h, d_pulse, d_q_in, d_q_out, stream, O.scratch_slot);
        if (rc) return rc;
    }
    if (!(stage & 2)) return WF_OK;
    WF_REQUIRE(ctx->d_mod_scratch != nullptr, "wf_mod_chan_bank: stage 2 without the carries of stage 1");
    double *const scratch_main = mod_scratch_of(ctx, P, O.scratch_slot);
    mcb_params Q;
    Q.rot_re = rot_re; Q.rot_im = rot_im; Q.sigma = sigma;
    Q.seed = seed; Q.stream_id = stream_id; Q.pair0 = first_index >> 1;
    Q.dyn_index = d_dyn_index;
    Q.k_lo = k_lo;
    Q.k_hi = k_lo + ncols;
    {
        const int64_t off = first - (cpm_nf ? sps / 2 : (mf_ntaps - 1) / 2);
        int64_t ks = off / sps;
        if (off - ks * sps < 0) --ks;
        Q.kshift = (int)ks;
        Q.d = (int)(off - ks * sps);
    }
    Q.mf_ntaps = mf_ntaps;
    Q.pack_par0 = pack_par0 & 1;
    Q.cpm_nh = cpm_nh;
    const int JM = J <= 4 ? 4 : 9;
    const int win = MOD_ROWS * (P.rs / sps) + JM + 2 + (pam ? 10 : 0);
    const int ring_slots = sps == 8 ? mcb_geom<8>::SLOTS : (sps == 10 ? mcb_geom<10>::SLOTS : mcb_geom<20>::SLOTS);
    const bool pam2 = pam && O.pam_factor != nullptr;
    if (pam2) {
        WF_REQUIRE((reinterpret_cast<uintptr_t>(O.pam_factor) & 7) == 0, "wf_mod_chan_bank: the bank's factorisation must be 8-byte aligned");
        d_mf_taps = O.pam_factor;
    }
    const size_t lds = (size_t)((win + 1) & ~1) * sizeof(double) + (size_t)(pam ? mcb_pam_slots(sps, pam2) : ring_slots) * sizeof(double2) +
                       (size_t)nh * (win + 1) * sizeof(int);
    int cus = 256;
    (void)hipDeviceGetAttribute(&cus, hipDeviceAttributeMultiprocessorCount, ctx->device);
#ifndef WF_MCB_TAIL_SLOTS_DEFAULT
#define WF_MCB_TAIL_SLOTS_DEFAULT 1.5
#endif
#ifndef WF_MCB_RUNS_PER_SLOT
#define WF_MCB_RUNS_PER_SLOT 4
#endif
#ifndef WF_MCB_RUNS_PER_SLOT_SOQPSK
#define WF_MCB_RUNS_PER_SLOT_SOQPSK 2
#endif
    const int runs_per_slot = cpm_nf ? (O.runs_hint > 0 ? O.runs_hint : WF_MCB_RUNS_PER_SLOT) : WF_MCB_RUNS_PER_SLOT_SOQPSK;
    const int64_t max_grid = (int64_t)cus * ((cpm_nf && JM != 4) || pam ? 3 : 4) * runs_per_slot;
    const int64_t per_run = (P.ntiles + max_grid - 1) / max_grid;
    const int64_t tail_opt = ctx->opt[WF_OPT_MCB_TAIL_PERMILLE];
    const double tail_slots = tail_opt == 0 ? WF_MCB_TAIL_SLOTS_DEFAULT : (tail_opt < 0 ? 0.0 : (double)tail_opt / 1000.0);
    int64_t tail = per_run > 1 && cpm_nf == 0 ? (int64_t)(tail_slots * (double)(max_grid / runs_per_slot)) : 0;
    if (tail > P.ntiles / 2) tail = P.ntiles / 2;
    Q.run_long = (int)per_run;
    Q.n_long = (int)((P.ntiles - tail) / per_run);
    const int grid = (int)(Q.n_long + (P.ntiles - (int64_t)Q.n_long * per_run));
    using kern_t = void (*)(const int8_t *, const double *, const double *, const double *, const double *, double *, mod_params, mcb_params);
    kern_t k = cpm_nf == 16 && O.cpm_paired && (JM != 4 || (P.c & 1) == 0) ? (JM == 4 ? mod_chan_bank_kernel<4, 32> : mod_chan_bank_kernel<9, 32>)
             : cpm_nf == 16 ? (JM == 4 ? mod_chan_bank_kernel<4, 16> : mod_chan_bank_kernel<9, 16>)
             : cpm_nf == 4 && O.cpm_paired ? (JM == 4 ? mod_chan_bank_kernel<4, 8> : mod_chan_bank_kernel<9, 8>)
             : cpm_nf == 4  ? (JM == 4 ? mod_chan_bank_kernel<4, 4> : mod_chan_bank_kernel<9, 4>)
             : pam2         ? (sps == 10 ? (JM == 4 ? mod_chan_bank_kernel<4, -2, 10> : mod_chan_bank_kernel<9, -2, 10>)
                                         : (JM == 4 ? mod_chan_bank_kernel<4, -2> : mod_chan_bank_kernel<9, -2>))
             : pam          ? (sps == 10 ? (JM == 4 ? mod_chan_bank_kernel<4, -1, 10> : mod_chan_bank_kernel<9, -1, 10>)
                                         : (JM == 4 ? mod_chan_bank_kernel<4, -1> : mod_chan_bank_kernel<9, -1>))
             : sps == 10    ? (JM == 4 ? mod_chan_bank_kernel<4, 0, 10> : mod_chan_bank_kernel<9, 0, 10>)
             : sps == 20    ? (JM == 4 ? mod_chan_bank_kernel<4, 0, 20> : mod_chan_bank_kernel<9, 0, 20>)
                            : (JM == 4 ? mod_chan_bank_kernel<4, 0> : mod_chan_bank_kernel<9, 0>);
    if (lds > 48 * 1024)
        WF_HIP(hipFuncSetAttribute(reinterpret_cast<const void *>(k), hipFuncAttributeMaxDynamicSharedMemorySize, (int)lds));
    hipLaunchKernelGGL(k, dim3(grid), dim3(MOD_THREADS), lds, wf_stream(stream), d_symbols, d_h, d_pulse, scratch_main, d_mf_taps,
                       d_rows4, P, Q);
    WF_LAUNCH_CHECK();
    return WF_OK;
}

int wf_mod_chan_bank_packed(wf_ctx *ctx, const int8_t *d_symbols, int64_t nsym, const double *d_h, int nh,
                            const double *d_pulse, int ntaps, int sps, double phi0, const double *d_mf_taps, double rot_re,
                            double rot_im, double sigma, uint64_t seed, uint64_t stream_id, uint64_t first_index,
                            int64_t first, int64_t ncols, int pack_par0, double *d_rows4, void *stream, int mf_ntaps, const wf_mcb_opts *opts,
                            int stage)
{
    return wf_mod_chan_bank_window(ctx, d_symbols, 0, nsym, nsym, d_h, nh, d_pulse, ntaps, sps, phi0, 0, -1, nullptr, nullptr, -1,
                                   d_mf_taps, rot_re, rot_im, sigma, seed, stream_id, first_index, nullptr, first, 0, ncols,
                                   pack_par0, d_rows4, stream, 0, 1, stage, mf_ntaps, opts);
}

int wf_mod_chan_bank_applies(int64_t nsym, int nh, int ntaps, int sps, int mf_ntaps, int64_t first)
{
    const bool pam = (sps == 8 || sps == 10) && mf_ntaps != sps + 1 && mf_ntaps >= 3 && mf_ntaps <= MCB_PAM_NT(sps) && (mf_ntaps & 1);
    if (!(sps == 8 || sps == 10 || sps == 20) || (mf_ntaps != sps + 1 && !pam) || first < 0 || first >= sps || nh < 1 || nh > 2) return 0;
    mod_params P;
    const int rs_want = sps == 8 ? mcb_geom<8>::RS : (sps == 10 ? mcb_geom<10>::RS : mcb_geom<20>::RS);
    if (!mod_setup(P, nsym, nh, ntaps, sps, 0.0) || P.rs != rs_want) return 0;
    if ((sps != 10 || (ntaps + sps - 1) / sps > 4) && ((sps & 1) || (P.c & 1))) return 0;
    return (ntaps + sps - 1) / sps <= 9;
}

int wf_mod_chan_cpm_rows_applies(int64_t nsym, int nh, int ntaps, int sps, int nfilt, int ntm, int64_t start0)
{
    if (ntm != 9 || start0 < -4 || start0 > 3 || (nfilt != 4 && nfilt != 16) || sps != 8 || (nh != 1 && nh != 2)) return 0;
    mod_params P;
    if (!mod_setup(P, nsym, nh, ntaps, sps, 0.0) || P.rs != 2 * MOD_THREADS) return 0;
    return (ntaps + sps - 1) / sps <= 9;
}

// ... 138 lines not shown
```

### waveforms_amd/csrc/wf_pipeline.hip

```cpp
#include "wf_common.h"

__global__ void time_axis_kernel(int64_t n, double step, double *__restrict__ out)
{
    const int64_t stride = (int64_t)gridDim.x * blockDim.x;
    for (int64_t k = (int64_t)blockIdx.x * blockDim.x + threadIdx.x; k < n; k += stride)
        out[k] = (double)k * step;
}

extern "C" int wf_time_axis_f64(wf_ctx *ctx, int64_t n, double step, double *d_out, void *stream)
{
    WF_REQUIRE(ctx && n >= 0, "wf_time_axis_f64: bad argument");
    if (n == 0) return WF_OK;
    WF_REQUIRE(d_out != nullptr, "wf_time_axis_f64: NULL output");
    WF_HIP(hipSetDevice(ctx->device));
    hipLaunchKernelGGL(time_axis_kernel, dim3(wf_grid_for(n, 256, 4096)), dim3(256), 0, wf_stream(stream), n,
                       step, d_out);
    WF_LAUNCH_CHECK();
    return WF_OK;
}

static inline int64_t round_up(int64_t v, int64_t a) { return (v + a - 1) / a * a; }

struct link_layout {
    int64_t nsym, npts, ncols, first;
    size_t off_bits, off_syms, off_freq, off_sig, off_mf, off_dbits, off_dsyms, total;
};

static link_layout make_layout(int64_t nsym, int sps, int ntaps, int nfilt, int length, int timing_offset)
{
    link_layout L;
    L.nsym = nsym;
    L.npts = wf_fir_out_len(nsym, sps, ntaps);
    const int64_t limit = L.npts - (int64_t)length * sps;
    int64_t first = (-(int64_t)timing_offset) % sps;
    if (first < 0) first += sps;
    L.first = first;
    L.ncols = limit > first ? (limit - first + sps - 1) / sps : 0;
    size_t o = 0;
    L.off_bits = o;  o += (size_t)round_up(nsym + 16, 256);
    L.off_syms = o;  o += (size_t)round_up(nsym + 16, 256);
    L.off_freq = o;  o += (size_t)round_up(L.npts * 8, 256);
    L.off_sig = o;   o += (size_t)round_up(L.npts * 16, 256);
    L.off_mf = o;    o += (size_t)round_up(L.ncols * nfilt * 16, 256);
    L.off_dbits = o; o += (size_t)round_up(L.ncols + 16, 256);
    L.off_dsyms = o; o += (size_t)round_up(L.ncols + 16, 256);
    L.total = o;
    return L;
}

static int link_warmup(const wf_link_config *cfg) { return cfg->warmup; }

static bool link_packed_rows8(const wf_link_config *cfg)
{
    return (cfg->fuse & 4) && (cfg->fuse & 2) && cfg->sps == 8 && cfg->mf_nfilt == 3;
}

static bool link_one_kernel(const wf_link_config *cfg)
{
    if ((cfg->fuse & 15) != 15 || cfg->mf_nfilt != 3 || cfg->sps < 2) return false;
    int64_t first = (-(int64_t)cfg->timing_offset) % cfg->sps;
    if (first < 0) first += cfg->sps;
    return wf_mod_chan_bank_applies(cfg->nsym, 1, cfg->ntaps, cfg->sps, cfg->mf_ntaps, first) != 0;
}

static bool link_packed_rows(const wf_link_config *cfg) { return link_packed_rows8(cfg) || link_one_kernel(cfg); }

static bool link_pipelined(const wf_link_config *cfg) { return (cfg->fuse & 32) && link_one_kernel(cfg); }

static bool link_factor_matches(const unsigned char *const *host, const size_t *, const void *arg)
{
    const int nt = *static_cast<const int *>(arg);
    const double *taps = reinterpret_cast<const double *>(host[0]);
    const double *b = reinterpret_cast<const double *>(host[1]);
    const double *G = b + 2 * nt;
    double big = 0.0, worst = 0.0;
    for (int s = 0; s < 3; ++s)
        for (int t = 0; t < nt; ++t) {
            const double re = G[4 * s] * b[t] + G[4 * s + 2] * b[nt + t], im = G[4 * s + 1] * b[t] + G[4 * s + 3] * b[nt + t];
            const double tr = taps[2 * (s * nt + t)], ti = taps[2 * (s * nt + t) + 1];
            const double d = hypot(re - tr, im - ti), m = hypot(tr, ti);
            if (!(d == d)) return false;
            if (d > worst) worst = d;
            if (m > big) big = m;
        }
    return worst <= 1e-12 * big;
}
static int link_check_factor(wf_ctx *ctx, const wf_link_config *cfg, void *stream)
{
    if (!cfg->d_mf_factor || cfg->mf_ntaps == cfg->sps + 1 || cfg->mf_nfilt != 3 || cfg->mf_ntaps < 1) return WF_OK;
    const int nt = cfg->mf_ntaps;
    const void *ptrs[2] = {cfg->d_mf_taps, cfg->d_mf_factor};
    const size_t nb[2] = {(size_t)3 * nt * 16, (size_t)(2 * nt + 12) * 8};
    return wf_promise_verified(ctx, 2, ptrs, nb, 2, stream, link_factor_matches, &nt,
                               "wf_link_config.d_mf_factor does not reproduce d_mf_taps (taps[s] != sum_k G[s][k] b_k to 1e-12)");
}

extern "C" int64_t wf_link_workspace_bytes(const wf_link_config *cfg)
{
    if (!cfg || cfg->nsym < 1 || cfg->sps < 1) return -1;
    const int64_t one = (int64_t)make_layout(cfg->nsym, cfg->sps, cfg->ntaps, cfg->mf_nfilt, 2, cfg->timing_offset).total;
    return link_pipelined(cfg) ? 2 * round_up(one, 256) : one;
}

static hipStream_t link_masked_stream(const wf_ctx *ctx, int reserve)
{
    hipStream_t s = nullptr;
    if (reserve > 0 && reserve < ctx->cus) {
        const int words = (ctx->cus + 31) / 32;
        std::vector<uint32_t> mask((size_t)words, 0u);
        for (int cu = reserve; cu < ctx->cus; ++cu) mask[(size_t)(cu / 32)] |= 1u << (cu % 32);
        if (hipExtStreamCreateWithCUMask(&s, (uint32_t)words, mask.data()) == hipSuccess) return s;
        (void)hipGetLastError();
        s = nullptr;
    }
    if (hipStreamCreateWithFlags(&s, hipStreamDefault) != hipSuccess) return nullptr;
    return s;
}

extern "C" int wf_link_run(wf_ctx *ctx, const wf_link_config *cfg, void *d_workspace, int64_t workspace_bytes,
                           int64_t *d_counts, int64_t *h_compared, void *stream)
{
    WF_REQUIRE(ctx && cfg && d_workspace && d_counts, "wf_link_run: NULL argument");
    WF_REQUIRE(cfg->nsym >= 1 && cfg->sps >= 1 && cfg->mf_nfilt == 3, "wf_link_run: bad configuration");
    WF_REQUIRE((reinterpret_cast<uintptr_t>(d_workspace) & 255) == 0, "wf_link_run: workspace must be 256-byte aligned");
    const int length = 2;
    const link_layout L = make_layout(cfg->nsym, cfg->sps, cfg->ntaps, cfg->mf_nfilt, length, cfg->timing_offset);
    WF_REQUIRE((int64_t)L.total <= workspace_bytes, "wf_link_run: workspace too small (%lld < %lld)",
               (long long)workspace_bytes, (long long)L.total);
    WF_REQUIRE(L.npts >= cfg->mf_ntaps, "wf_link_run: burst shorter than the matched filter");
    char *w = static_cast<char *>(d_workspace);
    const bool piped = link_pipelined(cfg) && L.ncols > 0;
    void *s_pro = stream, *s_main = stream;
    bool ahead = false;
    int slot = -1;
    if (piped) {
        const int64_t set_bytes = round_up((int64_t)L.total, 256);
        WF_REQUIRE(2 * set_bytes <= workspace_bytes, "wf_link_run: fuse bit 5 needs two sets of intermediates (%lld bytes)", (long long)(2 * set_bytes));
        WF_HIP(hipSetDevice(ctx->device));
        if (!ctx->pipe_stream) {
            hipStream_t ps;
            WF_HIP(hipStreamCreateWithFlags(&ps, hipStreamNonBlocking));
            ctx->pipe_stream = ps;
            WF_HIP(hipEventCreateWithFlags(&ctx->pipe_front, hipEventDisableTiming));
            for (int k = 0; k < 2; ++k) WF_HIP(hipEventCreateWithFlags(&ctx->pipe_done[k], hipEventDisableTiming));
        }
        w += (int64_t)ctx->pipe_set * set_bytes;
        const int64_t rsv = ctx->opt[WF_OPT_PIPE_RESERVE_CUS];
        ahead = rsv != 0;
        if (ahead) {
            if (!ctx->pipe_pro) {
                hipStream_t sp;
                WF_HIP(hipStreamCreateWithFlags(&sp, hipStreamDefault));
                ctx->pipe_pro = sp;
                ctx->pipe_main = link_masked_stream(ctx, rsv < 0 ? 0 : (int)rsv);
                WF_REQUIRE(ctx->pipe_main != nullptr, "wf_link_run: could not create the front end's stream");
                WF_HIP(hipEventCreateWithFlags(&ctx->pipe_call, hipEventDisableTiming));
                WF_HIP(hipEventCreateWithFlags(&ctx->pipe_pro_done, hipEventDisableTiming));
            }
            s_pro = ctx->pipe_pro;
            s_main = ctx->pipe_main;
            slot = ctx->pipe_set;
            if (stream) {
                WF_HIP(hipEventRecord(ctx->pipe_call, wf_stream(stream)));
                WF_HIP(hipStreamWaitEvent(wf_stream(s_pro), ctx->pipe_call, 0));
            }
            if (ctx->pipe_done_valid[ctx->pipe_set]) WF_HIP(hipStreamWaitEvent(wf_stream(s_pro), ctx->pipe_done[ctx->pipe_set], 0));
        } else if (ctx->pipe_done_valid[ctx->pipe_set]) {
            WF_HIP(hipStreamWaitEvent(wf_stream(stream), ctx->pipe_done[ctx->pipe_set], 0));
        }
    } else {
        const int rj = wf_link_join_internal(ctx, stream);
        if (rj) return rj;
    }
    uint8_t *bits = reinterpret_cast<uint8_t *>(w + L.off_bits);
    int8_t *syms = reinterpret_cast<int8_t *>(w + L.off_syms);
    double *freq = reinterpret_cast<double *>(w + L.off_freq);
    double *sig = reinterpret_cast<double *>(w + L.off_sig);
    double *mf = reinterpret_cast<double *>(w + L.off_mf);
    uint8_t *dbits = reinterpret_cast<uint8_t *>(w + L.off_dbits);
    int8_t *dsyms = reinterpret_cast<int8_t *>(w + L.off_dsyms);

    uint8_t next[2][4][2];
    int8_t outp[2][4][2];
    static const int8_t kOut[2][8] = {{0, 2, 0, -2, -2, 0, 2, 0}, {0, -2, 2, 0, 0, 2, -2, 0}};
    for (int c = 0; c < 2; ++c)
        for (int b = 0; b < 8; ++b) {
            const int s = b >> 1;
            const int e = c == 0 ? (s & 1) + 2 * (b & 1) : (s & 2) + (b & 1);
            const int flip = cfg->differential ? (c == 0 ? (s >> 1) : (s & 1)) : 0;
            const int inp = (b & 1) ^ flip;
            next[c][s][inp] = (uint8_t)e;
            outp[c][s][inp] = kOut[c][b];
        }
    hipEvent_t *ev = nullptr;
    if (cfg->event_slot >= 0) {
        WF_REQUIRE(cfg->event_slot < WF_LINK_EVENT_SLOTS, "wf_link_run: event_slot %d", cfg->event_slot);
        if (!ctx->events) {
            ctx->events = new hipEvent_t[WF_LINK_EVENT_SLOTS * (WF_LINK_STAGES + 1)];
            for (int k = 0; k < WF_LINK_EVENT_SLOTS * (WF_LINK_STAGES + 1); ++k) WF_HIP(hipEventCreate(&ctx->events[k]));
        }
        ev = ctx->events + cfg->event_slot * (WF_LINK_STAGES + 1);
    }
#define MARKS(k, s) do { if (ev) WF_HIP(hipEventRecord(ev[k], wf_stream(s))); } while (0)
#define MARK(k) MARKS(k, stream)
    int rc;
    MARKS(0, s_pro);
    rc = (cfg->fuse & 16) ? 1 : wf_soqpsk_prbs_encode(ctx, cfg->degree, cfg->mask, cfg->state, cfg->skip, &next[0][0][0], &outp[0][0][0], bits,
                                                       cfg->nsym, syms, s_pro, ev ? (void *)ev[1] : nullptr);
    if (rc < 0) return rc;
    if (rc == 1) {
        if ((rc = wf_lfsr_generate(ctx, cfg->degree, cfg->mask, cfg->state, cfg->skip, bits, cfg->nsym, nullptr, s_pro))) return rc;
        MARKS(1, s_pro);
        if ((rc = wf_fsm_encode(ctx, &next[0][0][0], &outp[0][0][0], 2, 4, 1, bits, cfg->nsym, 0, 0, syms, nullptr, s_pro))) return rc;
    }
    if (!ahead) MARKS(2, s_pro);
    bool fused_all = false;
    if (link_one_kernel(cfg) && L.ncols > 0) {
        wf_mcb_opts mo;
        mo.pam_factor = cfg->d_mf_factor;
        mo.scratch_slot = slot;
        if ((rc = link_check_factor(ctx, cfg, stream))) return rc;
        for (int stage = ahead ? 1 : 3; stage <= (ahead ? 2 : 3); ++stage) {
            if (ahead && stage == 2) {
                MARKS(2, s_pro);
                WF_HIP(hipEventRecord(ctx->pipe_pro_done, wf_stream(s_pro)));
                WF_HIP(hipStreamWaitEvent(wf_stream(s_main), ctx->pipe_pro_done, 0));
                MARKS(3, s_main);
            }
            rc = wf_mod_chan_bank_packed(ctx, syms, cfg->nsym, cfg->d_h, 1, cfg->d_pulse, cfg->ntaps, cfg->sps, M_PI / 4, cfg->d_mf_taps,
                                         cos(-M_PI / 4), sin(-M_PI / 4), cfg->sigma, cfg->seed, cfg->stream_id, 0, L.first, L.ncols, 0,
                                         mf, stage == 1 ? s_pro : s_main, cfg->mf_ntaps, &mo, stage);
            if (rc < 0) return rc;
            WF_REQUIRE(rc == 0, "wf_link_run: internal: the one-kernel front end refused a configuration wf_mod_chan_bank_applies accepted");
        }
        fused_all = true;
    }
    if (fused_all) {
        if (!ahead) MARKS(3, s_main);
        MARKS(4, s_main); MARKS(5, s_main);
        void *back = stream;
        if (piped) {
            back = ctx->pipe_stream;
            WF_HIP(hipEventRecord(ctx->pipe_front, wf_stream(s_main)));
            WF_HIP(hipStreamWaitEvent(wf_stream(back), ctx->pipe_front, 0));
        }
#define MARKB(k) do { if (ev) WF_HIP(hipEventRecord(ev[k], wf_stream(back))); } while (0)
        MARKB(6);
        rc = wf_viterbi4_detect_packed(ctx, mf, L.ncols, cfg->differential, link_warmup(cfg), dbits, dsyms, nullptr, back);
        if (rc) return rc;
        MARKB(7);
        int64_t m_ = L.ncols - length;
        if (m_ > cfg->nsym) m_ = cfg->nsym;
        if (m_ < 0) m_ = 0;
        if ((rc = wf_count_errors(ctx, dsyms + length, syms, dbits + length, bits, m_, d_counts, back))) return rc;
        MARKB(8);
#undef MARKB
        if (piped) {
            WF_HIP(hipEventRecord(ctx->pipe_done[ctx->pipe_set], wf_stream(back)));
            ctx->pipe_done_valid[ctx->pipe_set] = true;
            ctx->pipe_set ^= 1;
        }
        if (h_compared) *h_compared = m_;
        return WF_OK;
    }
    bool fused_mod = false;
    if (cfg->fuse & 1) {
        rc = wf_cpm_modulate_c128(ctx, syms, cfg->nsym, cfg->d_h, 1, cfg->d_pulse, cfg->ntaps, cfg->sps, M_PI / 4, sig, stream);
        if (rc < 0) return rc;
        fused_mod = rc == 0;
    }
    if (fused_mod) {
        MARK(3);
    } else {
        if ((rc = wf_upsample_fir_f64(ctx, syms, cfg->nsym, cfg->d_h, 1, cfg->d_pulse, cfg->ntaps, cfg->sps, freq, stream))) return rc;
        MARK(3);
        if ((rc = wf_phase_cexp_f64(ctx, freq, L.npts, cfg->sps, M_PI / 4, 0.0, sig, nullptr, stream))) return rc;
    }
    MARK(4);
    const double rot_re = cos(-M_PI / 4), rot_im = sin(-M_PI / 4);
    const bool fused_chan = (cfg->fuse & 2) && L.ncols > 0;
    if (!fused_chan)
        if ((rc = wf_awgn_c128(ctx, sig, L.npts, rot_re, rot_im, cfg->sigma, cfg->seed, cfg->stream_id, 0, sig, stream))) return rc;
    MARK(5);
    int64_t m = L.ncols - length;
    if (m > cfg->nsym) m = cfg->nsym;
    if (m < 0) m = 0;
    const bool fused_count = false;
    const bool packed = fused_chan && link_packed_rows8(cfg);
    if (L.ncols > 0) {
        if (packed)
            rc = wf_awgn_mf_bank_dyn(ctx, sig, L.npts, rot_re, rot_im, cfg->sigma, cfg->seed, cfg->stream_id, 0, nullptr,
                                     cfg->d_mf_taps, cfg->mf_nfilt, cfg->mf_ntaps, L.first, cfg->sps, L.ncols, mf, stream, 0);
        else if (fused_chan)
            rc = wf_awgn_mf_bank_c128(ctx, sig, L.npts, rot_re, rot_im, cfg->sigma, cfg->seed, cfg->stream_id, 0,
                                      cfg->d_mf_taps, cfg->mf_nfilt, cfg->mf_ntaps, L.first, cfg->sps, L.ncols, mf, stream);
        else
            rc = wf_mf_bank_c128(ctx, sig, L.npts, cfg->d_mf_taps, cfg->mf_nfilt, cfg->mf_ntaps, L.first, cfg->sps,
                                 L.ncols, mf, stream);
        if (rc) return rc;
        MARK(6);
        if (fused_count)
            rc = wf_viterbi4_detect_count(ctx, mf, L.ncols, cfg->differential, link_warmup(cfg), dbits, dsyms, bits, syms,
                                          length, m, d_counts, stream);
        else if (packed)
            rc = wf_viterbi4_detect_packed(ctx, mf, L.ncols, cfg->differential, link_warmup(cfg), dbits, dsyms, nullptr, stream);
        else
            rc = wf_viterbi4_detect(ctx, mf, L.ncols, cfg->differential, link_warmup(cfg), dbits, dsyms, nullptr, stream);
        if (rc) return rc;
    } else {
        MARK(6);
    }
    MARK(7);
    if (m > 0 && !fused_count)
        if ((rc = wf_count_errors(ctx, dsyms + length, syms, dbits + length, bits, m, d_counts, stream))) return rc;
    MARK(8);
#undef MARK
    if (h_compared) *h_compared = m;
    return WF_OK;
}

extern "C" int wf_link_stage_ms(wf_ctx *ctx, int event_slot, float *h_ms)
{
    WF_REQUIRE(ctx && h_ms && event_slot >= 0 && event_slot < WF_LINK_EVENT_SLOTS && ctx->events,
               "wf_link_stage_ms: no events recorded in slot %d", event_slot);
    hipEvent_t *ev = ctx->events + event_slot * (WF_LINK_STAGES + 1);
    WF_HIP(hipEventSynchronize(ev[WF_LINK_STAGES]));
    for (int k = 0; k < WF_LINK_STAGES; ++k) WF_HIP(hipEventElapsedTime(&h_ms[k], ev[k], ev[k + 1]));
    return WF_OK;
}

extern "C" int wf_link_layout(const wf_link_config *cfg, int64_t *info8)
{
    if (!cfg || !info8 || cfg->nsym < 1 || cfg->sps < 1) return WF_ERR_VALUE;
    const link_layout L = make_layout(cfg->nsym, cfg->sps, cfg->ntaps, cfg->mf_nfilt, 2, cfg->timing_offset);
    info8[0] = L.ncols; info8[2] = (int64_t)L.off_dbits; info8[3] = (int64_t)L.off_dsyms;
    info8[4] = (int64_t)L.off_sig; info8[6] = L.npts; info8[7] = (int64_t)L.off_mf;
    info8[1] = link_one_kernel(cfg) ? 1 : 0;
    info8[5] = link_packed_rows(cfg) ? 32 : 16 * cfg->mf_nfilt;
    return WF_OK;
}

struct stream_layout {
    int64_t N, B, c, tile_len, spt, ntiles_total, halo, npts, ncols_total, first, m_total;
    int64_t k_lo, ncols, ws, nloc, tile_lo, ntiles, out_origin, local_len, ws_next, q_out_tile;
    size_t off_bits, off_syms, off_sig, off_mf, off_dbits, off_dsyms, total;
    bool ok;
};

static stream_layout make_stream_layout(const wf_link_config *cfg, int64_t B, int64_t c)
{
    stream_layout S;
    const int length = 2;
    S.N = cfg->nsym; S.B = B; S.c = c;
    if (cfg->sps < 2 || cfg->sps > 256 || cfg->ntaps < 1 || cfg->nsym < 1 || cfg->mf_ntaps < 1) {
        S = stream_layout{};
        return S;
    }
    S.ok = wf_mod_tile_geometry(cfg->sps, cfg->ntaps, cfg->nsym, &S.tile_len, &S.spt, &S.ntiles_total) == 0;
    S.halo = round_up(S.spt + 48, 16);
    S.npts = wf_fir_out_len(S.N, cfg->sps, cfg->ntaps);
    const int64_t limit = S.npts - (int64_t)length * cfg->sps;
    int64_t first = (-(int64_t)cfg->timing_offset) % cfg->sps;
    if (first < 0) first += cfg->sps;
    S.first = first;
    S.ncols_total = limit > first ? (limit - first + cfg->sps - 1) / cfg->sps : 0;
    S.m_total = S.ncols_total - length < S.N ? S.ncols_total - length : S.N;
    if (S.m_total < 0) S.m_total = 0;
    S.ok = S.ok && B > 0 && B % S.spt == 0 && B % 128 == 0 && B >= 4 * S.halo &&
           S.tile_len >= cfg->mf_ntaps + 2 * cfg->sps;
    S.k_lo = c * B;
    const int64_t k_hi = S.k_lo + B < S.ncols_total ? S.k_lo + B : S.ncols_total;
    S.ncols = k_hi > S.k_lo ? k_hi - S.k_lo : 0;
    S.ws = c * B - S.halo > 0 ? c * B - S.halo : 0;
    const int64_t we = (c + 1) * B + S.halo < S.N ? (c + 1) * B + S.halo : S.N;
    S.nloc = we > S.ws ? we - S.ws : 0;
    S.tile_lo = S.spt > 0 && c * B / S.spt - 1 > 0 ? c * B / S.spt - 1 : 0;
    int64_t tile_hi = S.spt > 0 ? (c + 1) * B / S.spt + 1 : 0;
    if (tile_hi > S.ntiles_total) tile_hi = S.ntiles_total;
    S.ntiles = tile_hi > S.tile_lo ? tile_hi - S.tile_lo : 0;
    S.out_origin = S.tile_lo * S.tile_len;
    const int64_t hi = tile_hi * S.tile_len < S.npts ? tile_hi * S.tile_len : S.npts;
    S.local_len = hi > S.out_origin ? hi - S.out_origin : 0;
    S.ws_next = (c + 1) * B - S.halo > 0 ? (c + 1) * B - S.halo : 0;
    const int64_t next_tile_lo = S.spt > 0 ? (c + 1) * B / S.spt - 1 : 0;
    S.q_out_tile = (next_tile_lo >= S.tile_lo && next_tile_lo < tile_hi) ? next_tile_lo - S.tile_lo : -1;
    size_t o = 0;
    const int64_t win = B + 2 * S.halo + 32;
    S.off_bits = o;  o += (size_t)round_up(win, 256);
    S.off_syms = o;  o += (size_t)round_up(win, 256);
    S.off_sig = o;   o += (size_t)round_up((B * cfg->sps + 2 * S.tile_len) * 16, 256);
    S.off_mf = o;    o += (size_t)round_up(B * cfg->mf_nfilt * 16, 256);
    S.off_dbits = o; o += (size_t)round_up(B + 16, 256);
    S.off_dsyms = o; o += (size_t)round_up(B + 16, 256);
    S.total = o;
    return S;
}

extern "C" int64_t wf_link_stream_workspace_bytes(const wf_link_config *cfg, int64_t chunk_symbols)
{
    if (!cfg || cfg->nsym < 1 || cfg->sps < 2) return -1;
    const stream_layout S = make_stream_layout(cfg, chunk_symbols, 0);
    return S.ok ? (int64_t)S.total : -1;
}

extern "C" int wf_link_stream_layout(const wf_link_config *cfg, int64_t chunk_symbols, int64_t chunk_index, int64_t *info8)
{
    if (!cfg || !info8 || cfg->nsym < 1 || cfg->sps < 2) return WF_ERR_VALUE;
    const stream_layout S = make_stream_layout(cfg, chunk_symbols, chunk_index);
    if (!S.ok) return WF_ERR_VALUE;
    info8[0] = S.ncols; info8[1] = S.k_lo; info8[2] = (int64_t)S.off_dbits; info8[3] = (int64_t)S.off_dsyms;
// ... 170 lines not shown
```

### waveforms_amd/csrc/wf_viterbi.hip

```cpp
#include <stddef.h>
#include <stdlib.h>
#include <string.h>

#include <time.h>

#include "wf_viterbi4.h"

#define VIT_THREADS 256
#define VIT_DEFAULT_WARMUP 31
#define VIT_MAX_LEN 64

template <int COL>
__device__ __forceinline__ void vit_acs(const double m[4], const vit_comp &q, double out[4], uint64_t second[4])
{
    double fa[4], fb[4];
    if (COL == 0) {
        fa[0] = m[0] - q.i1; fb[0] = m[2] + q.a;
        fa[1] = m[1] - q.r1; fb[1] = m[3] + q.b;
        fa[2] = m[0] - q.b;  fb[2] = m[2] + q.r1;
        fa[3] = m[1] - q.a;  fb[3] = m[3] + q.i1;
    } else {
        fa[0] = m[0] - q.i1; fb[0] = m[1] - q.b;
        fa[1] = m[0] - q.a;  fb[1] = m[1] - q.r1;
        fa[2] = m[2] + q.r1; fb[2] = m[3] + q.a;
// ... 203 lines not shown
#pragma unroll
    for (int k = 0; k < 4; ++k) L.m0[k] = 0.0;
    L.prev.r1 = L.prev.i1 = L.prev.a = L.prev.b = 0.0;
    L.wb = L.ws = 0;
    if (state && a == 0) {
#pragma unroll
        for (int k = 0; k < 4; ++k) L.m0[k] = state[1 + k];
        L.prev = vit_comp_from_inc(state + 5, (int)((i0 - 1) & 1));
    }
#if VIT_DEPTH == 3
    double2 pend0[NP], pend1[NP], pend2[NP];
#else
    double2 pend0[NP], pend1[NP];
#endif
    const int last_b = nbatch - 1;
    fetch(0, pend0);
    fetch(min(1, last_b), pend1);
#if VIT_DEPTH == 3
    fetch(min(2, last_b), pend2);
#endif
    const int64_t kbase = a - warmup - 1;
    auto round = [&](int b, double2 (&pd)[NP]) __attribute__((always_inline)) {
        stash(pd);
        fetch(min(b + VIT_DEPTH, last_b), pd);
        __builtin_amdgcn_fence(__ATOMIC_RELEASE, "wavefront");
        __builtin_amdgcn_wave_barrier();
        __builtin_amdgcn_fence(__ATOMIC_ACQUIRE, "wavefront");
        if (live) {
#pragma unroll 1
            for (int jj = 0; jj < VIT_S; jj += 2) {
                const int j = b * VIT_S + jj;
                const int64_t k = kbase + j;
                const double2 *zr = tile + lane * LS + RW * jj;
                if (j == warmup + 1) vit_save_start(L);
                if (j < nsteps && k >= 0 && k < ncalls)
                    vit_step<PAR0, PACKED>(L, zr, j == 0, diff, k, a, ncalls, dec);
                if (j + 1 == warmup + 1) vit_save_start(L);
                if (j + 1 < nsteps && k + 1 >= 0 && k + 1 < ncalls)
                    vit_step<PAR0 ^ 1, PACKED>(L, zr + RW, false, diff, k + 1, a, ncalls, dec);
            }
        }
        __builtin_amdgcn_fence(__ATOMIC_RELEASE, "wavefront");
        __builtin_amdgcn_wave_barrier();
        __builtin_amdgcn_fence(__ATOMIC_ACQUIRE, "wavefront");
    };
    for (int b0 = 0; b0 < nbatch; b0 += VIT_DEPTH) {
        round(b0, pend0);
        round(b0 + 1, pend1);
#if VIT_DEPTH == 3
        round(b0 + 2, pend2);
#endif
    }
    if (live) vit_flush(dec, CH, a, ncalls, bits, syms);
    if (edge && live) {
        double *e = edge + 8 * (g0 + lane);
        *reinterpret_cast<double4 *>(e) = make_double4(L.ms[0], L.ms[1], L.ms[2], L.ms[3]);
        *reinterpret_cast<double4 *>(e + 4) = make_double4(L.m0[0], L.m0[1], L.m0[2], L.m0[3]);
    }
    if (state && live && a + CH >= ncalls) {
        state[16] = (double)(i0 + ncalls);
#pragma unroll
        for (int k = 0; k < 4; ++k) state[17 + k] = L.m0[k];
        vit_comp_to_inc(L.prev, (int)((i0 + ncalls - 1) & 1), state + 21);
    }
}

#ifndef VIT_MIN_WAVES
#define VIT_MIN_WAVES 1
#endif
template <bool PACKED>
__global__ __launch_bounds__(VIT_THREADS, VIT_MIN_WAVES) void viterbi_batch_kernel(const double *__restrict__ mf, int64_t ncalls,
                                                                     int ch, int diff, int warmup, uint8_t *__restrict__ bits,
                                                                     int8_t *__restrict__ syms, double *__restrict__ state,
                                                                     double *__restrict__ edge, int64_t nchunks)
{
    __shared__ double2 s_rows[VIT_THREADS / WF_WAVE][WF_WAVE * VIT_LANE_SLOTS];
    extern __shared__ uint64_t s_dec[];
    const int64_t i0 = state ? (int64_t)state[0] : 0;
    if (blockIdx.x == 0 && threadIdx.x < VIT_HDR) reinterpret_cast<uint64_t *>(edge + 8 * nchunks)[threadIdx.x] = 0;
    if ((i0 - warmup - 1) & 1) viterbi_batch_body<1, PACKED>(mf, ncalls, ch, diff, warmup, bits, syms, state, i0, s_rows, s_dec, edge);
    else viterbi_batch_body<0, PACKED>(mf, ncalls, ch, diff, warmup, bits, syms, state, i0, s_rows, s_dec, edge);
}

template <int PAR, bool PACKED>
__device__ __forceinline__ bool vit_rerun_chunk(const double *__restrict__ mf, int64_t ncalls, int CH, int diff, uint8_t *__restrict__ bits,
                                                int8_t *__restrict__ syms, double *__restrict__ state, int64_t i0, double *__restrict__ edge, int64_t c)
{
    constexpr int RW = PACKED ? 2 : 3;
    const double2 *rows = reinterpret_cast<const double2 *>(mf);
    const int64_t a = c * CH, kend = a + CH < ncalls ? a + CH : ncalls;
    double *rec = edge + 8 * c;
    vit_lane L;
    L.wb = L.ws = 0;
#pragma unroll
    for (int q = 0; q < 4; ++q) {
        const double v = __hip_atomic_load(rec - 4 + q, __ATOMIC_RELAXED, __HIP_MEMORY_SCOPE_AGENT);
        L.m0[q] = v;
        rec[q] = v;
    }
    L.prev = vit_components<PAR ^ 1, PACKED>(rows + RW * (a - 1));
    for (int64_t k = a; k < kend; k += 2) {
        bool bit, cd0, cd1;
        vit_step_core<PAR, PACKED>(L, rows + RW * k, diff, bit, cd0, cd1);
        bits[k] = bit ? 1 : 0;
        syms[k] = (int8_t)(2 * ((cd0 ? 1 : 0) | (cd1 ? 2 : 0)) - 2);
        if (k + 1 < kend) {
            vit_step_core<PAR ^ 1, PACKED>(L, rows + RW * (k + 1), diff, bit, cd0, cd1);
            bits[k + 1] = bit ? 1 : 0;
            syms[k + 1] = (int8_t)(2 * ((cd0 ? 1 : 0) | (cd1 ? 2 : 0)) - 2);
        }
    }
    bool changed = false;
#pragma unroll
    for (int q = 0; q < 4; ++q) {
        changed |= __double_as_longlong(rec[4 + q]) != __double_as_longlong(L.m0[q]);
        rec[4 + q] = L.m0[q];
    }
    if (changed && state && a + CH >= ncalls) {
#pragma unroll
        for (int q = 0; q < 4; ++q) state[17 + q] = L.m0[q];
    }
    return changed;
}

template <bool PACKED>
__global__ __launch_bounds__(256) void viterbi_fixup_kernel(const double *__restrict__ mf, int64_t ncalls, int ch, int diff,
                                                            uint8_t *__restrict__ bits, int8_t *__restrict__ syms, double *__restrict__ state,
                                                            double *__restrict__ edge, int64_t nchunks, unsigned long long *__restrict__ unmerged, int mode)
{
    if (!vit_fixup_verify(edge, nchunks, unmerged, mode)) return;
    const int64_t i0 = state ? (int64_t)state[0] : 0;
    if (i0 & 1)
        vit_fixup_rounds(edge, nchunks, unmerged, [&](int64_t c) { return vit_rerun_chunk<1, PACKED>(mf, ncalls, ch, diff, bits, syms, state, i0, edge, c); });
    else
        vit_fixup_rounds(edge, nchunks, unmerged, [&](int64_t c) { return vit_rerun_chunk<0, PACKED>(mf, ncalls, ch, diff, bits, syms, state, i0, edge, c); });
}

__global__ void viterbi_carry_commit_kernel(double *state)
{
    const int t = threadIdx.x;
    if (t < 16) state[t] = state[16 + t];
}

static int viterbi_launch(wf_ctx *ctx, const double *d_mf_ri, int64_t ncalls, int differential, int warmup,
                          uint8_t *d_bits, int8_t *d_syms, double *d_state, void *stream, bool packed = false)
{
    WF_REQUIRE(ctx && ncalls >= 0 && warmup >= 0, "wf_viterbi4_detect: bad argument");
    if (ncalls == 0) return WF_OK;
    WF_REQUIRE(d_mf_ri && d_bits && d_syms, "wf_viterbi4_detect: NULL device pointer");
    WF_REQUIRE((reinterpret_cast<uintptr_t>(d_mf_ri) & 15) == 0 && (reinterpret_cast<uintptr_t>(d_bits) & 15) == 0 &&
                   (reinterpret_cast<uintptr_t>(d_syms) & 15) == 0,
               "wf_viterbi4_detect: device pointers must be 16-byte aligned");
    WF_HIP(hipSetDevice(ctx->device));
    if (warmup == 0) warmup = VIT_DEFAULT_WARMUP;
    if (warmup > 4096) warmup = 4096;
#ifndef VIT_CHUNK_LANES
#define VIT_CHUNK_LANES 65536
#endif
    int ch = (int)((ncalls + VIT_CHUNK_LANES - 1) / VIT_CHUNK_LANES);
    ch = (ch + 15) / 16 * 16;
    if (ch < 32) ch = 32;
    if (ch > 512) ch = 512;
    const int64_t nthreads = (ncalls + ch - 1) / ch;
    const int64_t nblocks = (nthreads + VIT_THREADS - 1) / VIT_THREADS;
    WF_REQUIRE(nblocks < (1ll << 31), "wf_viterbi4_detect: burst too long for one launch");
    hipStream_t s = wf_stream(stream);
    const size_t lds = (size_t)VIT_THREADS * (ch / 16 + 1) * sizeof(uint64_t);
    int rcv = wf_ctx_reserve_vit(ctx, vit_edge_words(nthreads));
    if (rcv) return rcv;
    double *edge = ctx->d_vit_edge;
    if (lds > 32 * 1024) {
        const void *kfn = packed ? reinterpret_cast<const void *>(viterbi_batch_kernel<true>)
                                 : reinterpret_cast<const void *>(viterbi_batch_kernel<false>);
        WF_HIP(hipFuncSetAttribute(kfn, hipFuncAttributeMaxDynamicSharedMemorySize, (int)lds));
    }
    if (packed)
        hipLaunchKernelGGL(viterbi_batch_kernel<true>, dim3((unsigned)nblocks), dim3(VIT_THREADS), lds, s, d_mf_ri, ncalls, ch,
                           differential ? 1 : 0, warmup, d_bits, d_syms, d_state, edge, nthreads);
    else
        hipLaunchKernelGGL(viterbi_batch_kernel<false>, dim3((unsigned)nblocks), dim3(VIT_THREADS), lds, s, d_mf_ri, ncalls, ch,
                           differential ? 1 : 0, warmup, d_bits, d_syms, d_state, edge, nthreads);
    WF_LAUNCH_CHECK();
    if (nthreads > 1) {
        const unsigned fgrid = (unsigned)wf_grid_for(nthreads - 1, 256, 1024);
        const int passes = ctx->opt[WF_OPT_DET_REPAIR] == 0 && ctx->opt[WF_OPT_DET_FINAL_VERIFY] ? 2 : 1;
        for (int pass = 0; pass < passes; ++pass) {
            const int mode = pass == 0 && ctx->opt[WF_OPT_DET_REPAIR] == 0 ? 1 : 0;
            if (packed)
                hipLaunchKernelGGL(viterbi_fixup_kernel<true>, dim3(fgrid), dim3(256), 0, s, d_mf_ri, ncalls, ch, differential ? 1 : 0, d_bits, d_syms,
                                   d_state, edge, nthreads, ctx->d_vit_unmerged, mode);
            else
                hipLaunchKernelGGL(viterbi_fixup_kernel<false>, dim3(fgrid), dim3(256), 0, s, d_mf_ri, ncalls, ch, differential ? 1 : 0, d_bits, d_syms,
                                   d_state, edge, nthreads, ctx->d_vit_unmerged, mode);
            WF_LAUNCH_CHECK();
        }
    }
    if (d_state) {
        hipLaunchKernelGGL(viterbi_carry_commit_kernel, dim3(1), dim3(64), 0, s, d_state);
        WF_LAUNCH_CHECK();
    }
    return WF_OK;
}

extern "C" int wf_viterbi4_detect(wf_ctx *ctx, const double *d_mf_ri, int64_t ncalls, int differential,
                                  int warmup, uint8_t *d_bits, int8_t *d_syms, double *d_state,
                                  void *stream)
{
    return viterbi_launch(ctx, d_mf_ri, ncalls, differential, warmup, d_bits, d_syms, d_state, stream);
}

extern "C" int wf_viterbi4_unmerged(wf_ctx *ctx, int64_t *h_count, int reset, void *stream)
{
    WF_REQUIRE(ctx && h_count, "wf_viterbi4_unmerged: NULL argument");
    WF_HIP(hipSetDevice(ctx->device));
    hipStream_t s = wf_stream(stream);
    unsigned long long v = 0;
    WF_HIP(hipMemcpyAsync(&v, ctx->d_vit_unmerged, sizeof(v), hipMemcpyDeviceToHost, s));
    WF_HIP(hipStreamSynchronize(s));
    if (reset && v) WF_HIP(hipMemsetAsync(ctx->d_vit_unmerged, 0, sizeof(v), s));
    *h_count = (int64_t)v;
    return WF_OK;
}

extern "C" int wf_viterbi_repaired(wf_ctx *ctx, int64_t *h_count, int reset, void *stream)
{
    WF_REQUIRE(ctx && h_count, "wf_viterbi_repaired: NULL argument");
    WF_HIP(hipSetDevice(ctx->device));
    hipStream_t s = wf_stream(stream);
    unsigned long long v = 0;
    WF_HIP(hipMemcpyAsync(&v, ctx->d_vit_unmerged + 1, sizeof(v), hipMemcpyDeviceToHost, s));
    WF_HIP(hipStreamSynchronize(s));
    if (reset && v) WF_HIP(hipMemsetAsync(ctx->d_vit_unmerged + 1, 0, sizeof(v), s));
    *h_count = (int64_t)v;
    return WF_OK;
}

extern "C" int wf_viterbi_cascaded(wf_ctx *ctx, int64_t *h_count, int reset, void *stream)
{
    WF_REQUIRE(ctx && h_count, "wf_viterbi_cascaded: NULL argument");
    WF_HIP(hipSetDevice(ctx->device));
    hipStream_t s = wf_stream(stream);
    unsigned long long v = 0;
    WF_HIP(hipMemcpyAsync(&v, ctx->d_vit_unmerged + 2, sizeof(v), hipMemcpyDeviceToHost, s));
    WF_HIP(hipStreamSynchronize(s));
    if (reset && v) WF_HIP(hipMemsetAsync(ctx->d_vit_unmerged + 2, 0, sizeof(v), s));
    *h_count = (int64_t)v;
    return WF_OK;
}

int wf_viterbi4_detect_packed(wf_ctx *ctx, const double *d_rows4, int64_t ncalls, int differential, int warmup,
                              uint8_t *d_bits, int8_t *d_syms, double *d_state, void *stream)
{
    return viterbi_launch(ctx, d_rows4, ncalls, differential, warmup, d_bits, d_syms, d_state, stream, true);
}

extern "C" int wf_viterbi4_detect_count(wf_ctx *ctx, const double *d_mf_ri, int64_t ncalls, int differential,
                                        int warmup, uint8_t *d_bits, int8_t *d_syms, const uint8_t *d_ref_bits,
                                        const int8_t *d_ref_syms, int skip, int64_t ncompare, int64_t *d_counts,
                                        void *stream)
{
    WF_REQUIRE(d_ref_bits && d_ref_syms && d_counts && skip >= 0 && ncompare >= 0,
               "wf_viterbi4_detect_count: bad reference arguments");
    int rc = viterbi_launch(ctx, d_mf_ri, ncalls, differential, warmup, d_bits, d_syms, nullptr, stream);
    if (rc) return rc;
    int64_t m = ncalls - skip;
    if (m > ncompare) m = ncompare;
    if (m <= 0) return WF_OK;
    return wf_count_errors(ctx, d_syms + skip, d_ref_syms, d_bits + skip, d_ref_bits, m, d_counts, stream);
}

#define VWIN_THREADS 128
#define VWIN_MAX_LEN VIT_MAX_LEN
#define VWIN_STATE_DOUBLES 1024
#define VWIN_STAGE 512
static_assert(8 + 4 * (VWIN_MAX_LEN - 1) <= VWIN_STAGE, "carry block");

template <int COL>
__device__ __forceinline__ void vwin_acs(const double m[4], const vit_comp &q, double out[4], bool lt[4])
{
    double fa[4], fb[4];
    if (COL == 0) {
        fa[0] = m[0] - q.i1; fb[0] = m[2] + q.a;
        fa[1] = m[1] - q.r1; fb[1] = m[3] + q.b;
        fa[2] = m[0] - q.b;  fb[2] = m[2] + q.r1;
        fa[3] = m[1] - q.a;  fb[3] = m[3] + q.i1;
    } else {
        fa[0] = m[0] - q.i1; fb[0] = m[1] - q.b;
        fa[1] = m[0] - q.a;  fb[1] = m[1] - q.r1;
        fa[2] = m[2] + q.r1; fb[2] = m[3] + q.a;
        fa[3] = m[2] + q.b;  fb[3] = m[3] + q.i1;
    }
#pragma unroll
    for (int s = 0; s < 4; ++s) {
        lt[s] = fb[s] < fa[s];
        out[s] = lt[s] ? fb[s] : fa[s];
    }
}

__device__ __forceinline__ uint32_t vwin_code(int col, int e, int second, int diff)
{
    const int start = col == 0 ? (e & 1) + 2 * second : (e & 2) + second;
    const int b = 2 * start + (col == 0 ? e >> 1 : e & 1);
    return (uint32_t)br_inp(col, b, diff) | ((uint32_t)br_out_idx(col, b) << 1);
}

template <int COL>
__device__ __forceinline__ void vwin_stage(double m[4], uint32_t d[4], const vit_comp &q, bool first, int diff)
{
    double o[4];
    bool lt[4];
    vwin_acs<COL>(m, q, o, lt);
    uint32_t n[4];
    if (first) {
#pragma unroll
        for (int e = 0; e < 4; ++e) n[e] = lt[e] ? vwin_code(COL, e, 1, diff) : vwin_code(COL, e, 0, diff);
    } else if (COL == 0) {
        n[0] = lt[0] ? d[2] : d[0]; n[1] = lt[1] ? d[3] : d[1]; n[2] = lt[2] ? d[2] : d[0]; n[3] = lt[3] ? d[3] : d[1];
    } else {
        n[0] = lt[0] ? d[1] : d[0]; n[1] = lt[1] ? d[1] : d[0]; n[2] = lt[2] ? d[3] : d[2]; n[3] = lt[3] ? d[3] : d[2];
    }
#pragma unroll
    for (int e = 0; e < 4; ++e) {
        m[e] = o[e];
        d[e] = n[e];
    }
}

template <int CR>
__device__ __forceinline__ double vwin_inc(int b, const vit_comp &q)
{
    if (CR == 0) {
        switch (b) {
        case 0: return -q.i1; case 1: return -q.b; case 2: return -q.r1; case 3: return -q.a;
        case 4: return q.a; case 5: return q.r1; case 6: return q.b; default: return q.i1;
        }
    }
// ... 705 lines not shown
```

### waveforms_amd/csrc/wf_viterbi4.h

```cpp
#pragma once

#include "wf_common.h"

__device__ __forceinline__ int br_out_idx(int col, int b) { return (int)((0x49616419u >> (2 * (8 * col + b))) & 3u); }

__device__ __forceinline__ int br_end(int col, int b)
{
    const int s = b >> 1;
    return col == 0 ? (s & 1) + 2 * (b & 1) : (s & 2) + (b & 1);
}

__device__ __forceinline__ int br_inp(int col, int b, int diff)
{
    const int s = b >> 1;
    const int flip = diff ? (col == 0 ? (s >> 1) : (s & 1)) : 0;
    return (b & 1) ^ flip;
}

__device__ __forceinline__ double br_inc(int start, double re, double im)
{
    return start == 0 ? -im : start == 1 ? -re : start == 2 ? re : im;
}

struct vit_comp {
    double r1, i1, a, b;
};

template <int COL, bool PACKED>
__device__ __forceinline__ vit_comp vit_components(const double2 *__restrict__ z)
{
    vit_comp c;
    if (PACKED) {
        c.r1 = z[0].x;
        c.i1 = z[0].y;
        c.a = z[1].x;
        c.b = z[1].y;
        return c;
    }
    c.r1 = z[1].x;
    c.i1 = z[1].y;
    c.a = COL == 0 ? z[0].x : z[0].y;
    c.b = COL == 0 ? z[2].y : z[2].x;
    return c;
}

#define VIT_HDR 8
__host__ __device__ inline size_t vit_edge_words(int64_t nchunks) { return (size_t)nchunks * 8 + VIT_HDR + 2 * (size_t)nchunks; }

__device__ __forceinline__ bool vit_fixup_verify(double *__restrict__ edge, int64_t nchunks, unsigned long long *__restrict__ unmerged, int mode)
{
    __shared__ int s_last;
    unsigned long long *hdr = reinterpret_cast<unsigned long long *>(edge + 8 * nchunks);
    unsigned long long *list0 = hdr + VIT_HDR;
    const unsigned long long *rec = reinterpret_cast<const unsigned long long *>(edge);
    int listed = 0;
    for (int64_t c = (int64_t)blockIdx.x * blockDim.x + threadIdx.x + 1; c < nchunks; c += (int64_t)gridDim.x * blockDim.x) {
        const unsigned long long *st = rec + 8 * c, *en = rec + 8 * (c - 1) + 4;
        if (st[0] != en[0] || st[1] != en[1] || st[2] != en[2] || st[3] != en[3]) {
            if (mode) list0[atomicAdd(&hdr[0], 1ull)] = (unsigned long long)c;
            else atomicAdd(unmerged, 1ull);
            listed = 1;
        }
    }
    if (!mode) return false;
    if (__syncthreads_or(listed)) __threadfence();
    __syncthreads();
    if (threadIdx.x == 0) s_last = atomicAdd(&hdr[2], 1ull) + 1 == (unsigned long long)gridDim.x;
    __syncthreads();
    if (!s_last) return false;
    if (__hip_atomic_load(&hdr[0], __ATOMIC_RELAXED, __HIP_MEMORY_SCOPE_AGENT) == 0) return false;
    __threadfence();
    return true;
}

template <class F>
__device__ __forceinline__ void vit_fixup_rounds(double *__restrict__ edge, int64_t nchunks, unsigned long long *__restrict__ unmerged, F &&repair)
{
    unsigned long long *hdr = reinterpret_cast<unsigned long long *>(edge + 8 * nchunks);
    int lin = 0;
    for (;;) {
        const int64_t n = (int64_t)__hip_atomic_load(&hdr[lin], __ATOMIC_RELAXED, __HIP_MEMORY_SCOPE_AGENT);
        if (n == 0) return;
        unsigned long long *in = hdr + VIT_HDR + (int64_t)lin * nchunks, *out = hdr + VIT_HDR + (int64_t)(lin ^ 1) * nchunks;
        for (int64_t idx = threadIdx.x; idx < n; idx += blockDim.x) {
            const int64_t c = (int64_t)__hip_atomic_load(&in[idx], __ATOMIC_RELAXED, __HIP_MEMORY_SCOPE_AGENT);
            const bool changed = repair(c);
            atomicAdd(unmerged + 1, 1ull);
            if (changed) {
                atomicAdd(unmerged + 2, 1ull);
                if (c + 1 < nchunks) out[atomicAdd(&hdr[lin ^ 1], 1ull)] = (unsigned long long)(c + 1);
            }
        }
        __threadfence();
        __syncthreads();
        if (threadIdx.x == 0) __hip_atomic_store(&hdr[lin], 0ull, __ATOMIC_RELAXED, __HIP_MEMORY_SCOPE_AGENT);
        __threadfence();
        __syncthreads();
        lin ^= 1;
    }
}
```

### waveforms_amd/link.py

```python
from __future__ import annotations

import ctypes
import math

import numpy as np

from . import _hip
from .cpm.soqpsk import freq_pulse_soqpsk_tg
from .filters.matched import pack_bank_factors, pam_bank_factors, pam_matched_filter_taps, pt_matched_filter_taps
from .glfsr.pn import generate_mask


def sigma_for_ebn0(ebn0_db: float, sps: int) -> float:
    return math.sqrt(sps / (2.0 * 10.0 ** (ebn0_db / 10.0)))


def operating_point_warmup(waveform: str, ebn0_db: float | None) -> int:
    if ebn0_db is None:
        return 0
    if waveform == "soqpsk":
        return 16 if ebn0_db >= 6.0 else 0
    if waveform == "multih":
        return 48 if ebn0_db >= 8.0 else (64 if ebn0_db >= 6.0 else 0)
    return 64 if ebn0_db >= 3.0 else 0
# ... 8 lines not shown
        self._configure(nsym, sps, **kw)
        self.workspace_bytes = _hip.lib().wf_link_workspace_bytes(ctypes.byref(self.cfg))
        if self.workspace_bytes < 0:
            raise ValueError("invalid link configuration")
        self.workspace = _hip.empty(self.workspace_bytes, "uint8")
        self.counts = _hip.zeros(2, "int64")
        self.compared = 0

    def _configure(self, nsym: int, sps: int = 8, pulse=None, mod_index: float = 0.25, detector: str = "PT",
                   pn_degree: int = 23, differential: bool = True, timing_offset: int | None = None,
                   warmup: int = 0, fuse: int = 15, private_ctx: bool = False, factor_bank: bool = True) -> None:
        self.nsym, self.sps = int(nsym), int(sps)
        self._ctx = _hip.new_ctx() if private_ctx else _hip.ctx()
        _hip.check(_hip.lib().wf_ctx_forget_promises(self._ctx))
        self._owns_ctx = bool(private_ctx)
        pulse = freq_pulse_soqpsk_tg(sps) if pulse is None else np.asarray(pulse, dtype=np.float64)
        factors = None
        if detector == "PT":
            taps = pt_matched_filter_taps(pulse, mod_index, sps)
            off = -1 if timing_offset is None else timing_offset
        elif detector == "PAM":
            taps = pam_matched_filter_taps(pulse, mod_index, sps)
            off = 0 if timing_offset is None else timing_offset
            if factor_bank:
                factors = pam_bank_factors(pulse, mod_index, sps)
                if np.abs(factors[1] @ factors[0] - taps).max() > 1e-12 * np.abs(taps).max():
                    factors = None
        else:
            raise ValueError(f"unknown detector {detector!r}")
        self.detector = detector
        self.pn_degree = pn_degree
        self._d_h = _hip.to_device(np.array([mod_index], dtype=np.float64))
        self._d_pulse = _hip.to_device(pulse)
        self._d_taps = _hip.to_device(np.ascontiguousarray(taps))
        cfg = _hip.LinkConfig()
        cfg.nsym, cfg.sps = self.nsym, self.sps
        cfg.degree, cfg.mask, cfg.state, cfg.skip = pn_degree, generate_mask(pn_degree), (1 << pn_degree) - 1, 0
        cfg.differential = int(differential)
        cfg.d_h, cfg.d_pulse, cfg.ntaps = self._d_h.data_ptr(), self._d_pulse.data_ptr(), pulse.size
        cfg.d_mf_taps, cfg.mf_ntaps, cfg.mf_nfilt = self._d_taps.data_ptr(), taps.shape[1], taps.shape[0]
        cfg.timing_offset, cfg.warmup = off, warmup
        cfg.sigma, cfg.seed, cfg.stream_id = 0.0, 1, 0
        cfg.event_slot = -1
        cfg.fuse = int(fuse)
        self._d_factor = _hip.to_device(pack_bank_factors(*factors)) if factors is not None else None
        cfg.d_mf_factor = self._d_factor.data_ptr() if self._d_factor is not None else None
        self.cfg = cfg

    def __del__(self):
        try:
            if getattr(self, "cfg", None) is not None and (self.cfg.fuse & 32) and getattr(self, "workspace", None) is not None:
                _hip.lib().wf_link_join(self._ctx, _hip.stream())
                _hip.torch().cuda.current_stream().synchronize()
        except Exception:
            pass
        if getattr(self, "_owns_ctx", False):
            _hip.free_ctx(self._ctx)
            self._owns_ctx = False

    @property
    def row_bytes(self) -> int:
        return self.layout()["row_bytes"]

    def layout(self) -> dict:
        info = (ctypes.c_int64 * 8)()
        _hip.check(_hip.lib().wf_link_layout(ctypes.byref(self.cfg), info))
        keys = ("calls", "one_kernel_front_end", "off_bits", "off_syms", "off_signal", "row_bytes", "signal_len", "off_mf")
        return dict(zip(keys, (int(v) for v in info)))

    def reset_counts(self) -> None:
        _hip.check(_hip.lib().wf_link_join(self._ctx, _hip.stream()))
        self.counts.zero_()
        self.compared = 0

    STAGES = ("prbs", "encode", "fir", "phase", "awgn", "mfbank", "viterbi", "count")

    def stage_ms(self, event_slot: int) -> dict[str, float]:
        buf = (ctypes.c_float * len(self.STAGES))()
        _hip.check(_hip.lib().wf_link_stage_ms(self._ctx, event_slot, buf))
        d = dict(zip(self.STAGES, (float(v) for v in buf)))
        if self.prologue_ahead:
            d["fir"], d["phase"] = d["phase"], 0.0
        return d

    @property
    def prologue_ahead(self) -> bool:
        return bool(self.cfg.fuse & 32) and bool(self.layout()["one_kernel_front_end"]) and _hip.get_option(self._ctx, _hip.WF_OPT_PIPE_RESERVE_CUS) != 0

    def run_block(self, ebn0_db: float, seed: int = 1, stream_id: int = 0, skip_bits: int = 0,
                  event_slot: int = -1) -> None:
        c = self.cfg
        c.sigma, c.seed, c.stream_id, c.skip = sigma_for_ebn0(ebn0_db, self.sps), seed, stream_id, skip_bits
        c.event_slot = event_slot
        m = ctypes.c_int64(0)
        _hip.check(_hip.lib().wf_link_run(self._ctx, ctypes.byref(c), self.workspace.data_ptr(),
                                          self.workspace_bytes, self.counts.data_ptr(), ctypes.byref(m),
                                          _hip.stream()))
        self.compared += m.value

    def result(self) -> tuple[int, int, int]:
        _hip.check(_hip.lib().wf_ctx_check(self._ctx, _hip.stream()))
        from waveforms_amd import device as dev

        unmerged = dev.viterbi_unmerged(reset=True, ctx=self._ctx)
        if unmerged:
            raise RuntimeError(f"{unmerged} detector chunk(s) were left unproven (the repairs are switched off on this context)")
        se, be = (int(v) for v in self.counts.cpu().tolist())
        return se, be, self.compared


class SOQPSKStream:

    @property
    def row_bytes(self) -> int:
        c = self.cfg
        return 32 if (c.fuse & 4) and (c.fuse & 2) and c.sps == 8 and c.mf_nfilt == 3 else 16 * c.mf_nfilt

    def __init__(self, total_symbols: int, chunk_symbols: int, sps: int = 8, **kw) -> None:
        self._proto = SOQPSKLink.__new__(SOQPSKLink)
        SOQPSKLink._configure(self._proto, int(total_symbols), sps, **kw)
        self.cfg, self._ctx, self.sps = self._proto.cfg, self._proto._ctx, int(sps)
        self.total_symbols, self.chunk_symbols = int(total_symbols), int(chunk_symbols)
        lib = _hip.lib()
        nbytes = lib.wf_link_stream_workspace_bytes(ctypes.byref(self.cfg), self.chunk_symbols)
        if nbytes < 0:
            tl, spt, nt = ctypes.c_int64(), ctypes.c_int64(), ctypes.c_int64()
            lib.wf_mod_tile_geometry(self.sps, self.cfg.ntaps, self.total_symbols, ctypes.byref(tl), ctypes.byref(spt),
                                     ctypes.byref(nt))
            raise ValueError(f"chunk_symbols must be a multiple of {spt.value} (one modulator tile) and of 128, and at "
                             f"least {4 * (spt.value + 48)}")
        self.workspace_bytes = nbytes
        self.workspace = _hip.empty(nbytes, "uint8")
        self.state = _hip.zeros(64, "float64")
        self.counts = _hip.zeros(2, "int64")
        self.compared = 0
        info = (ctypes.c_int64 * 8)()
        _hip.check(lib.wf_link_layout(ctypes.byref(self.cfg), info))
        self.total_calls = int(info[0])
        self.nchunks = -(-self.total_calls // self.chunk_symbols)

    def reset(self) -> None:
        self.state.zero_()
        self.counts.zero_()
        self.compared = 0

    def chunk_info(self, c: int) -> dict:
        info = (ctypes.c_int64 * 8)()
        _hip.check(_hip.lib().wf_link_stream_layout(ctypes.byref(self.cfg), self.chunk_symbols, c, info))
        keys = ("calls", "first_call", "off_bits", "off_syms", "off_signal", "signal_origin", "signal_len", "off_mf")
        return dict(zip(keys, (int(v) for v in info)))

    def run_chunk(self, c: int, ebn0_db: float, seed: int = 1, stream_id: int = 0) -> None:
        cfg = self.cfg
        cfg.sigma, cfg.seed, cfg.stream_id, cfg.event_slot = sigma_for_ebn0(ebn0_db, self.sps), seed, stream_id, -1
        m = ctypes.c_int64(0)
        _hip.check(_hip.lib().wf_link_stream_chunk(self._ctx, ctypes.byref(cfg), self.chunk_symbols, c,
                                                   self.state.data_ptr(), self.workspace.data_ptr(), self.workspace_bytes,
                                                   self.counts.data_ptr(), ctypes.byref(m), _hip.stream()))
        self.compared += m.value

    def run(self, ebn0_db: float, seed: int = 1, stream_id: int = 0) -> tuple[int, int, int]:
        self.reset()
        for c in range(self.nchunks):
            self.run_chunk(c, ebn0_db, seed, stream_id)
        return self.result()

# ... 339 lines not shown
```

Measured before the change: 21840 Msym/s.

## Write matched-filter rows lane-major and add a one-chunk-per-lane Viterbi detector

The fused modulator/matched-filter kernel can now store its packed 4-column rows in a lane-major interleaved layout (chunk index in the low 6 bits), so the 64 lanes of a wavefront read consecutive rows of their own chunks with coalesced 32-byte loads. A new Viterbi kernel runs one chunk per lane with a 4-deep register prefetch of rows and warm-up rows taken from the previous chunk. The fixup/repair kernel is templated on a row-address function so it can re-run chunks in the lane-major layout. The path is gated by a new context option and a workspace-size check, and it adds complex address arithmetic in the store path (magic-number division) plus larger LDS use per block for decisions.

```diff
diff --git a/include/wfhip.h b/include/wfhip.h
--- a/include/wfhip.h
+++ b/include/wfhip.h
@@ -36,7 +36,8 @@
     WF_OPT_CPM_SAMPLES_MIN_CALLS = 7,
     WF_OPT_SOFT_CHUNK_CALLS = 8,
     WF_OPT_CPM_SOFT_CHUNK_CALLS = 9,
-    WF_OPT_COUNT = 10
+    WF_OPT_LINK_LANE_ROWS = 10,
+    WF_OPT_COUNT = 11
 } wf_option;
 int wf_ctx_set_option(wf_ctx *ctx, int key, int64_t value);
 int wf_ctx_get_option(wf_ctx *ctx, int key, int64_t *value);
@@ -155,6 +156,7 @@
 int wf_link_join(wf_ctx *ctx, void *stream);
 
 int wf_link_layout(const wf_link_config *cfg, int64_t *info8);
+int wf_link_lane_chunk(wf_ctx *ctx, const wf_link_config *cfg, int *h_chunk);
 
 #define WF_LINK_STREAM_STATE_BYTES 512
 int wf_mod_tile_geometry(int sps, int ntaps, int64_t nsym_total, int64_t *tile_len, int64_t *sym_per_tile,
diff --git a/waveforms_amd/_hip.py b/waveforms_amd/_hip.py
--- a/waveforms_amd/_hip.py
+++ b/waveforms_amd/_hip.py
@@ -15,7 +15,7 @@
 WF_CPM_STATE_BYTES, WF_CPM_STREAM_STATE_BYTES = 16384, 20480
 (WF_OPT_CPM_FORM, WF_OPT_CPM_CHUNK_CALLS, WF_OPT_DET_REPAIR, WF_OPT_DET_FINAL_VERIFY, WF_OPT_ITERATION_SERVER,
  WF_OPT_MCB_TAIL_PERMILLE, WF_OPT_PIPE_RESERVE_CUS, WF_OPT_CPM_SAMPLES_MIN_CALLS, WF_OPT_SOFT_CHUNK_CALLS,
- WF_OPT_CPM_SOFT_CHUNK_CALLS) = range(10)
+ WF_OPT_CPM_SOFT_CHUNK_CALLS, WF_OPT_LINK_LANE_ROWS) = range(11)
 
 _P = c_void_p
 SIGNATURES = {
@@ -65,6 +65,7 @@
     "wf_link_run": (c_int, [_P, _P, _P, c_int64, _P, POINTER(c_int64), _P]),
     "wf_link_stage_ms": (c_int, [_P, c_int, POINTER(ctypes.c_float)]),
     "wf_link_layout": (c_int, [_P, POINTER(c_int64)]),
+    "wf_link_lane_chunk": (c_int, [_P, _P, POINTER(c_int)]),
     "wf_mod_tile_geometry": (c_int, [c_int, c_int, c_int64, POINTER(c_int64), POINTER(c_int64), POINTER(c_int64)]),
     "wf_link_stream_workspace_bytes": (c_int64, [_P, c_int64]),
     "wf_link_stream_layout": (c_int, [_P, c_int64, c_int64, POINTER(c_int64)]),
diff --git a/waveforms_amd/csrc/wf_common.h b/waveforms_amd/csrc/wf_common.h
--- a/waveforms_amd/csrc/wf_common.h
+++ b/waveforms_amd/csrc/wf_common.h
@@ -109,6 +109,9 @@
                         int step, int64_t ncols, double *d_out_ri, void *stream, int pack_par0 = -1);
 int wf_viterbi4_detect_packed(wf_ctx *ctx, const double *d_rows4, int64_t ncalls, int differential, int warmup,
                               uint8_t *d_bits, int8_t *d_syms, double *d_state, void *stream);
+int64_t wf_viterbi4_lane_bytes(int64_t ncalls, int ch, int warmup);
+int wf_viterbi4_detect_lanes(wf_ctx *ctx, const double *d_rows4, int64_t ncalls, int ch, int differential, int warmup,
+                             uint8_t *d_bits, int8_t *d_syms, void *stream);
 int wf_cpm_modulate_window(wf_ctx *ctx, const int8_t *d_symbols, int64_t sym_origin, int64_t nloc, int64_t nsym_total,
                            const double *d_h, int nh, const double *d_pulse, int ntaps, int sps, double phi0,
                            int64_t tile_lo, int64_t ntiles, double *d_out_ri, int64_t out_origin,
@@ -118,6 +121,7 @@
     bool cpm_paired = false;
     int runs_hint = 0;
     int scratch_slot = -1;
+    int lane_ch = 0;
 };
 int wf_mod_chan_bank_packed(wf_ctx *ctx, const int8_t *d_symbols, int64_t nsym, const double *d_h, int nh,
                             const double *d_pulse, int ntaps, int sps, double phi0, const double *d_mf_taps, double rot_re,
diff --git a/waveforms_amd/csrc/wf_ctx.hip b/waveforms_amd/csrc/wf_ctx.hip
--- a/waveforms_amd/csrc/wf_ctx.hip
+++ b/waveforms_amd/csrc/wf_ctx.hip
@@ -122,6 +122,7 @@
     case WF_OPT_CPM_SAMPLES_MIN_CALLS: ok = value == 0 || (value >= 4096 && value <= ((int64_t)1 << 40)); break;
     case WF_OPT_SOFT_CHUNK_CALLS: ok = value >= 0 && value <= 8192; break;
     case WF_OPT_CPM_SOFT_CHUNK_CALLS: ok = value >= 0 && value <= 8192; break;
+    case WF_OPT_LINK_LANE_ROWS: ok = value == -1 || value == 0 || value == 1 || (value >= 64 && value <= 512 && value % 64 == 0); break;
     }
     WF_REQUIRE(ok, "wf_ctx_set_option: value %lld outside the range of option %d", (long long)value, key);
     c->opt[key] = value;
diff --git a/waveforms_amd/csrc/wf_modulate.hip b/waveforms_amd/csrc/wf_modulate.hip
--- a/waveforms_amd/csrc/wf_modulate.hip
+++ b/waveforms_amd/csrc/wf_modulate.hip
@@ -486,6 +486,8 @@
     int cpm_nh;
     int mf_ntaps;
     int n_long, run_long;
+    int lane_q;
+    unsigned lane_magic;
 };
 
 template <int SPS>
@@ -792,6 +794,26 @@
         const uint64_t *Wq = reinterpret_cast<const uint64_t *>(kt->scratch + MOD_OFF_P + P.ntiles);
         const double W = (double)Wq[ltile] * 0x1.0p-62 * P.sps_d;
         const int ref_a = s_pi[lpart], ref_b = P.nh > 1 ? s_pi[win + 1 + lpart] : 0;
+        auto store_packed = [&](int rho, bool k_ok, int slot, double val) __attribute__((always_inline)) {
+            if constexpr (SPS == 8 && CPMNF == 0) {
+                if (Q.lane_q) {
+                    const int q = Q.lane_q;
+                    const unsigned x = (unsigned)((int)(sym_base >> 6) + rho + q);
+                    const int gq = (int)(((uint64_t)x * Q.lane_magic) >> 31);
+                    const int r = (int)x - gq * q;
+                    const int g = gq - 1;
+                    const int e = mq - Q.kshift;
+                    const int64_t sa = ((int64_t)(g >> 6) * (64 * q) + 64 * r) * 64 + (g & 63);
+                    const unsigned KB = 32u * 4096u * (unsigned)(q - 1);
+                    const unsigned dw = (g & 63) == 63 ? KB + 32u * 4033u : 32u;
+                    char *const base = reinterpret_cast<char *>(rows) + 32 * sa - (int64_t)KB;
+                    const unsigned off = (r == q - 1 && e == 64 ? dw : KB + 2048u * (unsigned)e) + 8u * (unsigned)slot;
+                    if (k_ok) *reinterpret_cast<double *>(base + off) = val;
+                    return;
+                }
+            }
+            if (k_ok) *reinterpret_cast<double *>(tile_rows4 + (int64_t)(32 * (CPR * rho - Q.kshift)) + (unsigned)(32 * mq + 8 * slot)) = val;
+        };
         auto bank_row = [&](int rho) __attribute__((always_inline)) {
             const int kr = CPR * rho + mq - Q.kshift;
             const int64_t k = sym_base + kr;
@@ -928,9 +950,7 @@
                 }
                 const double T = S + mcb_quad_bcast<0xB1>(S);
                 const double val = (mp == 0 || mp == 3) ? U : T;
-                if (k_ok) {
-                    *reinterpret_cast<double *>(tile_rows4 + (int64_t)(32 * (CPR * rho - Q.kshift)) + (unsigned)(32 * mq + 8 * slot_l)) = val;
-                }
+                store_packed(rho, k_ok, slot_l, val);
             } else {
                 const int f = mp < 2 ? 1 : (mp == 2 ? 0 : 2);
                 const bool imag = mp == 1 || (mp == 2 && odd) || (mp == 3 && !odd);
@@ -942,7 +962,7 @@
                     const double2 tp = s_taps[f * NT + (NT - 1 - j)];
                     acc = imag ? fma(x.x, tp.y, fma(x.y, tp.x, acc)) : fma(x.x, tp.x, fma(-x.y, tp.y, acc));
                 }
-                if (k_ok) *reinterpret_cast<double *>(tile_rows4 + (int64_t)(32 * (CPR * rho - Q.kshift)) + (unsigned)(32 * mq + 8 * mp)) = acc;
+                store_packed(rho, k_ok, mp, acc);
             }
         };
         auto bank_reduce = [&](int rho) __attribute__((always_inline)) {
@@ -1371,6 +1391,14 @@
         Q.d = (int)(off - ks * sps);
     }
     Q.mf_ntaps = mf_ntaps;
+    Q.lane_q = 0;
+    Q.lane_magic = 0;
+    if (O.lane_ch) {
+        WF_REQUIRE(cpm_nf == 0 && !pam && sps == 8 && k_lo == 0 && O.lane_ch >= 64 && O.lane_ch <= 512 && O.lane_ch % 64 == 0 && ncols <= ((int64_t)1 << 30),
+                   "wf_mod_chan_bank: lane-major rows outside their form (chunk %d)", O.lane_ch);
+        Q.lane_q = O.lane_ch / 64;
+        Q.lane_magic = (unsigned)((((uint64_t)1 << 31) + (uint64_t)Q.lane_q - 1) / (uint64_t)Q.lane_q);
+    }
     Q.pack_par0 = pack_par0 & 1;
     Q.cpm_nh = cpm_nh;
     const int JM = J <= 4 ? 4 : 9;
diff --git a/waveforms_amd/csrc/wf_pipeline.hip b/waveforms_amd/csrc/wf_pipeline.hip
--- a/waveforms_amd/csrc/wf_pipeline.hip
+++ b/waveforms_amd/csrc/wf_pipeline.hip
@@ -93,6 +93,20 @@
     const size_t nb[2] = {(size_t)3 * nt * 16, (size_t)(2 * nt + 12) * 8};
     return wf_promise_verified(ctx, 2, ptrs, nb, 2, stream, link_factor_matches, &nt,
                                "wf_link_config.d_mf_factor does not reproduce d_mf_taps (taps[s] != sum_k G[s][k] b_k to 1e-12)");
+}
+
+static int link_lane_ch(const wf_ctx *ctx, const wf_link_config *cfg, const link_layout &L)
+{
+    const int64_t v = ctx->opt[WF_OPT_LINK_LANE_ROWS];
+    if (v <= 0) return 0;
+    if (cfg->sps != 8 || cfg->mf_ntaps != 9 || cfg->mf_nfilt != 3) return 0;
+    const int64_t have = round_up(L.ncols * cfg->mf_nfilt * 16, 256);
+    for (int ch = v >= 64 ? (int)v : (L.ncols >= ((int64_t)1 << 20) ? 128 : 64); ch <= 512; ch += 64) {
+        const int64_t need = wf_viterbi4_lane_bytes(L.ncols, ch, link_warmup(cfg));
+        if (need > 0) return need <= have ? ch : 0;
+        if (v >= 64) break;
+    }
+    return 0;
 }
 
 extern "C" int64_t wf_link_workspace_bytes(const wf_link_config *cfg)
@@ -215,10 +229,13 @@
     }
     if (!ahead) MARKS(2, s_pro);
     bool fused_all = false;
+    int lane_ch = 0;
     if (link_one_kernel(cfg) && L.ncols > 0) {
+        lane_ch = link_lane_ch(ctx, cfg, L);
         wf_mcb_opts mo;
         mo.pam_factor = cfg->d_mf_factor;
         mo.scratch_slot = slot;
+        mo.lane_ch = lane_ch;
         if ((rc = link_check_factor(ctx, cfg, stream))) return rc;
         for (int stage = ahead ? 1 : 3; stage <= (ahead ? 2 : 3); ++stage) {
             if (ahead && stage == 2) {
@@ -246,7 +263,8 @@
         }
 #define MARKB(k) do { if (ev) WF_HIP(hipEventRecord(ev[k], wf_stream(back))); } while (0)
         MARKB(6);
-        rc = wf_viterbi4_detect_packed(ctx, mf, L.ncols, cfg->differential, link_warmup(cfg), dbits, dsyms, nullptr, back);
+        rc = lane_ch ? wf_viterbi4_detect_lanes(ctx, mf, L.ncols, lane_ch, cfg->differential, link_warmup(cfg), dbits, dsyms, back)
+                     : wf_viterbi4_detect_packed(ctx, mf, L.ncols, cfg->differential, link_warmup(cfg), dbits, dsyms, nullptr, back);
         if (rc) return rc;
         MARKB(7);
         int64_t m_ = L.ncols - length;
@@ -326,6 +344,14 @@
     hipEvent_t *ev = ctx->events + event_slot * (WF_LINK_STAGES + 1);
     WF_HIP(hipEventSynchronize(ev[WF_LINK_STAGES]));
     for (int k = 0; k < WF_LINK_STAGES; ++k) WF_HIP(hipEventElapsedTime(&h_ms[k], ev[k], ev[k + 1]));
+    return WF_OK;
+}
+
+extern "C" int wf_link_lane_chunk(wf_ctx *ctx, const wf_link_config *cfg, int *h_chunk)
+{
+    WF_REQUIRE(ctx && cfg && h_chunk && cfg->nsym >= 1 && cfg->sps >= 1, "wf_link_lane_chunk: bad argument");
+    const link_layout L = make_layout(cfg->nsym, cfg->sps, cfg->ntaps, cfg->mf_nfilt, 2, cfg->timing_offset);
+    *h_chunk = link_one_kernel(cfg) && L.ncols > 0 ? link_lane_ch(ctx, cfg, L) : 0;
     return WF_OK;
 }
 
diff --git a/waveforms_amd/csrc/wf_viterbi.hip b/waveforms_amd/csrc/wf_viterbi.hip
--- a/waveforms_amd/csrc/wf_viterbi.hip
+++ b/waveforms_amd/csrc/wf_viterbi.hip
@@ -309,12 +309,74 @@
     else viterbi_batch_body<0, PACKED>(mf, ncalls, ch, diff, warmup, bits, syms, state, i0, s_rows, s_dec, edge);
 }
 
-template <int PAR, bool PACKED>
-__device__ __forceinline__ bool vit_rerun_chunk(const double *__restrict__ mf, int64_t ncalls, int CH, int diff, uint8_t *__restrict__ bits,
+#define VITL_PF 4
+
+template <int PAR0>
+__device__ __forceinline__ void viterbi_lanes_body(const double *__restrict__ mf, int64_t ncalls, int CH, int diff, int warmup,
+                                                   uint8_t *__restrict__ bits, int8_t *__restrict__ syms,
+                                                   uint64_t *__restrict__ s_dec, double *__restrict__ edge, int64_t nchunks)
+{
+    const int lane = threadIdx.x & 63, wave = threadIdx.x >> 6;
+    const int64_t B = (int64_t)__builtin_amdgcn_readfirstlane((int)(blockIdx.x * (VIT_THREADS / WF_WAVE) + wave));
+    if (B * WF_WAVE >= nchunks) return;
+    const int64_t a = (B * WF_WAVE + lane) * CH;
+    const bool live = a < ncalls;
+    const int W1 = warmup + 1, nsteps = W1 + CH, last = nsteps - 1;
+    uint64_t *dec = s_dec + (wave * WF_WAVE + lane) * (CH / 16 + 1);
+    const unsigned sh = B ? (unsigned)(WF_WAVE * CH) : 0u;
+    const char *lo = reinterpret_cast<const char *>(mf) + 32 * (B * WF_WAVE * (int64_t)CH - (int64_t)sh);
+    const unsigned own0 = 32u * (sh + (unsigned)lane) - 2048u * (unsigned)W1;
+    const unsigned wrm0 = lane ? 32u * (sh + (unsigned)(WF_WAVE * CH - 1 + lane)) - 2048u * (unsigned)W1
+                               : (B ? 32u * (sh + 63u) - 2048u * (unsigned)W1 : 0u);
+    auto fetch = [&](int s, double2 &z0, double2 &z1) __attribute__((always_inline)) {
+        const char *p = lo + ((s < W1 ? wrm0 : own0) + 2048u * (unsigned)s);
+        z0 = vit_ld16(reinterpret_cast<const double2 *>(p));
+        z1 = vit_ld16(reinterpret_cast<const double2 *>(p + 16));
+    };
+    vit_lane L;
+#pragma unroll
+    for (int k = 0; k < 4; ++k) L.m0[k] = 0.0;
+    L.prev.r1 = L.prev.i1 = L.prev.a = L.prev.b = 0.0;
+    L.wb = L.ws = 0;
+    double2 p0[VITL_PF], p1[VITL_PF];
+#pragma unroll
+    for (int u = 0; u < VITL_PF; ++u) fetch(min(u, last), p0[u], p1[u]);
+    const int64_t kbase = a - W1;
+    for (int s0 = 0; s0 < nsteps; s0 += VITL_PF) {
+#pragma unroll
+        for (int u = 0; u < VITL_PF; ++u) {
+            const int s = s0 + u;
+            const double2 z[2] = {p0[u], p1[u]};
+            fetch(min(s + VITL_PF, last), p0[u], p1[u]);
+            if (s == W1) vit_save_start(L);
+            const int64_t k = kbase + s;
+            if (live && s < nsteps && k >= 0 && k < ncalls) {
+                if (u & 1) vit_step<PAR0 ^ 1, true>(L, z, false, diff, k, a, ncalls, dec);
+                else vit_step<PAR0, true>(L, z, s == 0, diff, k, a, ncalls, dec);
+            }
+        }
+    }
+    if (!live) return;
+    vit_flush(dec, CH, a, ncalls, bits, syms);
+    double *e = edge + 8 * (B * WF_WAVE + lane);
+    *reinterpret_cast<double4 *>(e) = make_double4(L.ms[0], L.ms[1], L.ms[2], L.ms[3]);
+    *reinterpret_cast<double4 *>(e + 4) = make_double4(L.m0[0], L.m0[1], L.m0[2], L.m0[3]);
+}
+
+__global__ __launch_bounds__(VIT_THREADS, 4) void viterbi_lanes_kernel(const double *__restrict__ mf, int64_t ncalls, int ch, int diff, int warmup,
+                                                                       uint8_t *__restrict__ bits, int8_t *__restrict__ syms,
+                                                                       double *__restrict__ edge, int64_t nchunks)
+{
+    extern __shared__ uint64_t s_dec[];
+    if (blockIdx.x == 0 && threadIdx.x < VIT_HDR) reinterpret_cast<uint64_t *>(edge + 8 * nchunks)[threadIdx.x] = 0;
+    if ((warmup + 1) & 1) viterbi_lanes_body<1>(mf, ncalls, ch, diff, warmup, bits, syms, s_dec, edge, nchunks);
+    else viterbi_lanes_body<0>(mf, ncalls, ch, diff, warmup, bits, syms, s_dec, edge, nchunks);
+}
+
+template <int PAR, bool PACKED, class ROWAT>
+__device__ __forceinline__ bool vit_rerun_chunk(ROWAT &&row_at, int64_t ncalls, int CH, int diff, uint8_t *__restrict__ bits,
                                                 int8_t *__restrict__ syms, double *__restrict__ state, int64_t i0, double *__restrict__ edge, int64_t c)
 {
-    constexpr int RW = PACKED ? 2 : 3;
-    const double2 *rows = reinterpret_cast<const double2 *>(mf);
     const int64_t a = c * CH, kend = a + CH < ncalls ? a + CH : ncalls;
     double *rec = edge + 8 * c;
     vit_lane L;
@@ -325,14 +387,14 @@
         L.m0[q] = v;
         rec[q] = v;
     }
-    L.prev = vit_components<PAR ^ 1, PACKED>(rows + RW * (a - 1));
+    L.prev = vit_components<PAR ^ 1, PACKED>(row_at(a - 1));
     for (int64_t k = a; k < kend; k += 2) {
         bool bit, cd0, cd1;
-        vit_step_core<PAR, PACKED>(L, rows + RW * k, diff, bit, cd0, cd1);
+        vit_step_core<PAR, PACKED>(L, row_at(k), diff, bit, cd0, cd1);
         bits[k] = bit ? 1 : 0;
         syms[k] = (int8_t)(2 * ((cd0 ? 1 : 0) | (cd1 ? 2 : 0)) - 2);
         if (k + 1 < kend) {
-            vit_step_core<PAR ^ 1, PACKED>(L, rows + RW * (k + 1), diff, bit, cd0, cd1);
+            vit_step_core<PAR ^ 1, PACKED>(L, row_at(k + 1), diff, bit, cd0, cd1);
             bits[k + 1] = bit ? 1 : 0;
             syms[k + 1] = (int8_t)(2 * ((cd0 ? 1 : 0) | (cd1 ? 2 : 0)) - 2);
         }
@@ -357,10 +419,24 @@
 {
     if (!vit_fixup_verify(edge, nchunks, unmerged, mode)) return;
     const int64_t i0 = state ? (int64_t)state[0] : 0;
+    const double2 *rows = reinterpret_cast<const double2 *>(mf);
+    auto row_at = [&](int64_t k) { return rows + (PACKED ? 2 : 3) * k; };
     if (i0 & 1)
-        vit_fixup_rounds(edge, nchunks, unmerged, [&](int64_t c) { return vit_rerun_chunk<1, PACKED>(mf, ncalls, ch, diff, bits, syms, state, i0, edge, c); });
+        vit_fixup_rounds(edge, nchunks, unmerged, [&](int64_t c) { return vit_rerun_chunk<1, PACKED>(row_at, ncalls, ch, diff, bits, syms, state, i0, edge, c); });
     else
-        vit_fixup_rounds(edge, nchunks, unmerged, [&](int64_t c) { return vit_rerun_chunk<0, PACKED>(mf, ncalls, ch, diff, bits, syms, state, i0, edge, c); });
+        vit_fixup_rounds(edge, nchunks, unmerged, [&](int64_t c) { return vit_rerun_chunk<0, PACKED>(row_at, ncalls, ch, diff, bits, syms, state, i0, edge, c); });
+}
+
+template <bool PACKED, int LANE_MAJOR>
+__global__ __launch_bounds__(256) void viterbi_fixup_kernel(const double *__restrict__ mf, int64_t ncalls, int ch, int diff,
+                                                            uint8_t *__restrict__ bits, int8_t *__restrict__ syms,
+                                                            double *__restrict__ edge, int64_t nchunks, unsigned long long *__restrict__ unmerged, int mode)
+{
+    static_assert(PACKED && LANE_MAJOR == 1, "lane-major rows are packed rows");
+    if (!vit_fixup_verify(edge, nchunks, unmerged, mode)) return;
+    const double2 *rows = reinterpret_cast<const double2 *>(mf);
+    auto row_at = [&](int64_t k) { return rows + 2 * vit_lane_slot(k, ch); };
+    vit_fixup_rounds(edge, nchunks, unmerged, [&](int64_t c) { return vit_rerun_chunk<0, true>(row_at, ncalls, ch, diff, bits, syms, nullptr, 0, edge, c); });
 }
 
 __global__ void viterbi_carry_commit_kernel(double *state)
@@ -479,6 +555,51 @@
                               uint8_t *d_bits, int8_t *d_syms, double *d_state, void *stream)
 {
     return viterbi_launch(ctx, d_rows4, ncalls, differential, warmup, d_bits, d_syms, d_state, stream, true);
+}
+
+int64_t wf_viterbi4_lane_bytes(int64_t ncalls, int ch, int warmup)
+{
+    if (warmup == 0) warmup = VIT_DEFAULT_WARMUP;
+    if (ch < 64 || ch > 512 || ch % 64 || warmup < 0 || warmup + 1 > ch || ncalls < 64 || ncalls > ((int64_t)1 << 30)) return 0;
+    const int64_t nchunks = (ncalls + ch - 1) / ch;
+    return (nchunks + WF_WAVE - 1) / WF_WAVE * WF_WAVE * ch * 32;
+}
+
+int wf_viterbi4_detect_lanes(wf_ctx *ctx, const double *d_rows4, int64_t ncalls, int ch, int differential, int warmup,
+                             uint8_t *d_bits, int8_t *d_syms, void *stream)
+{
+    WF_REQUIRE(ctx && d_rows4 && d_bits && d_syms, "wf_viterbi4_detect_lanes: NULL argument");
+    WF_REQUIRE(wf_viterbi4_lane_bytes(ncalls, ch, warmup) > 0, "wf_viterbi4_detect_lanes: no lane-major form for %lld calls in chunks of %d, warm-up %d",
+               (long long)ncalls, ch, warmup);
+    WF_REQUIRE((reinterpret_cast<uintptr_t>(d_rows4) & 15) == 0 && (reinterpret_cast<uintptr_t>(d_bits) & 15) == 0 &&
+                   (reinterpret_cast<uintptr_t>(d_syms) & 15) == 0,
+               "wf_viterbi4_detect_lanes: device pointers must be 16-byte aligned");
+    WF_HIP(hipSetDevice(ctx->device));
+    if (warmup == 0) warmup = VIT_DEFAULT_WARMUP;
+    const int64_t nchunks = (ncalls + ch - 1) / ch;
+    const int64_t nwaves = (nchunks + WF_WAVE - 1) / WF_WAVE;
+    const int64_t nblocks = (nwaves * WF_WAVE + VIT_THREADS - 1) / VIT_THREADS;
+    hipStream_t s = wf_stream(stream);
+    const size_t lds = (size_t)VIT_THREADS * (ch / 16 + 1) * sizeof(uint64_t);
+    int rcv = wf_ctx_reserve_vit(ctx, vit_edge_words(nchunks));
+    if (rcv) return rcv;
+    double *edge = ctx->d_vit_edge;
+    if (lds > 32 * 1024)
+        WF_HIP(hipFuncSetAttribute(reinterpret_cast<const void *>(viterbi_lanes_kernel), hipFuncAttributeMaxDynamicSharedMemorySize, (int)lds));
+    hipLaunchKernelGGL(viterbi_lanes_kernel, dim3((unsigned)nblocks), dim3(VIT_THREADS), lds, s, d_rows4, ncalls, ch, differential ? 1 : 0, warmup,
+                       d_bits, d_syms, edge, nchunks);
+    WF_LAUNCH_CHECK();
+    if (nchunks > 1) {
+        const unsigned fgrid = (unsigned)wf_grid_for(nchunks - 1, 256, 1024);
+        const int passes = ctx->opt[WF_OPT_DET_REPAIR] == 0 && ctx->opt[WF_OPT_DET_FINAL_VERIFY] ? 2 : 1;
+        for (int pass = 0; pass < passes; ++pass) {
+            const int mode = pass == 0 && ctx->opt[WF_OPT_DET_REPAIR] == 0 ? 1 : 0;
+            hipLaunchKernelGGL((viterbi_fixup_kernel<true, 1>), dim3(fgrid), dim3(256), 0, s, d_rows4, ncalls, ch, differential ? 1 : 0, d_bits, d_syms,
+                               edge, nchunks, ctx->d_vit_unmerged, mode);
+            WF_LAUNCH_CHECK();
+        }
+    }
+    return WF_OK;
 }
 
 extern "C" int wf_viterbi4_detect_count(wf_ctx *ctx, const double *d_mf_ri, int64_t ncalls, int differential,
diff --git a/waveforms_amd/csrc/wf_viterbi4.h b/waveforms_amd/csrc/wf_viterbi4.h
--- a/waveforms_amd/csrc/wf_viterbi4.h
+++ b/waveforms_amd/csrc/wf_viterbi4.h
@@ -42,6 +42,12 @@
     c.a = COL == 0 ? z[0].x : z[0].y;
     c.b = COL == 0 ? z[2].y : z[2].x;
     return c;
+}
+
+__host__ __device__ inline int64_t vit_lane_slot(int64_t k, int CH)
+{
+    const int64_t g = k / CH;
+    return ((g >> 6) * CH + (k - g * CH)) * 64 + (g & 63);
 }
 
 #define VIT_HDR 8
diff --git a/waveforms_amd/link.py b/waveforms_amd/link.py
--- a/waveforms_amd/link.py
+++ b/waveforms_amd/link.py
@@ -114,6 +114,12 @@
         if self.prologue_ahead:
             d["fir"], d["phase"] = d["phase"], 0.0
         return d
+
+    @property
+    def lane_chunk(self) -> int:
+        ch = ctypes.c_int(0)
+        _hip.check(_hip.lib().wf_link_lane_chunk(self._ctx, ctypes.byref(self.cfg), ctypes.byref(ch)))
+        return int(ch.value)
 
     @property
     def prologue_ahead(self) -> bool:
```

After: 21480 Msym/s. -1.7%, worse.
